# ziyamammadov/conjugate-gradient-pyopencl

Measured on AMD Instinct MI355X. Metric: CG iterations/sec + SpMV effective HBM GB/s (% of 8 TB/s peak), N=10M CSR, higher is better.
Workload: dtype f64; 1 GPU; 3D 7-pt Laplacian 250x200x200 CSR, N=10000000, nnz=69720000, f64, 1 RHS, b=5, x0=0, fixed-iteration CG (fused 4-launch loop); rows=10000000, nnz=69720000, parallelism=1 GPU

## Files before the change

conjugate-gradient-pyopencl_amd/_lib.py:

```python
import ctypes
import os

import numpy as np

_HERE = os.path.dirname(os.path.abspath(__file__))
LIB_PATH = os.path.join(_HERE, "libcgamd.so")
LEGACY_LIB_PATH = os.path.join(_HERE, "liboclcg.so")

F32, F64, C64, C128 = 0, 1, 2, 3
DTYPE_CODE = {np.dtype(np.float32): F32, np.dtype(np.float64): F64,
              np.dtype(np.complex64): C64, np.dtype(np.complex128): C128}
CODE_DTYPE = {v: k for k, v in DTYPE_CODE.items()}

MATRIX_ON_DEVICE, NO_GRAPH, UNFUSED, DIST_GRAPH, DIST_NO_OVERLAP, DIST_P2P, DIST_P2P_STAGED, DIST_SINGLE_REDUCTION, DIST_RESIDENT = 1, 2, 4, 8, 32, 64, 128, 256, 512
HERMITIAN = 16
OK, ERR_INVALID, ERR_NO_DEVICE, ERR_HIP, ERR_ALLOC, ERR_IO, ERR_COMM, ERR_STATE = range(8)


class CgAmdError(RuntimeError):
    def __init__(self, status, message):
        super().__init__(f"cgamd status {status}: {message}")
        self.status = status


# ... 5 lines not shown
    if _lib is not None:
        return _lib
    if os.environ.get("CGAMD_NO_TORCH", "0") != "1":
        try:
            import torch
        except ImportError:
            pass
    if not os.path.exists(LIB_PATH):
        raise ImportError(
            f"{LIB_PATH} not found: the HIP extension is not built. Run `python -c 'import __graft_entry__ as g; "
            f"g.build()'` or `make -C {os.path.join(_HERE, 'csrc')}`. This package has no CPU fallback.")
    lib = ctypes.CDLL(LIB_PATH)
    vp, ci, ll, sz = ctypes.c_void_p, ctypes.c_int, ctypes.c_longlong, ctypes.c_size_t
    pvp = ctypes.POINTER(ctypes.c_void_p)
    sig = {
        "cgamd_last_error": (ctypes.c_char_p, []),
        "cgamd_version": (ci, []),
        "cgamd_dtype_size": (sz, [ci]),
        "cgamd_tune": (ci, [ctypes.c_char_p, ci]),
        "cgamd_device_count": (ci, []),
        "cgamd_device_name": (ci, [ci, ctypes.c_char_p, sz]),
        "cgamd_ctx_create": (ci, [ci, pvp]),
        "cgamd_ctx_destroy": (ci, [vp]),
        "cgamd_ctx_set_stream": (ci, [vp, vp]),
        "cgamd_ctx_stream": (vp, [vp]),
        "cgamd_ctx_device": (ci, [vp]),
        "cgamd_ctx_synchronize": (ci, [vp]),
        "cgamd_malloc": (ci, [vp, sz, pvp]),
        "cgamd_free": (ci, [vp, vp]),
        "cgamd_memcpy_h2d": (ci, [vp, vp, vp, sz]),
        "cgamd_memcpy_d2h": (ci, [vp, vp, vp, sz]),
        "cgamd_memcpy_d2d": (ci, [vp, vp, vp, sz]),
        "cgamd_memset": (ci, [vp, vp, ci, sz]),
        "cgamd_spmv": (ci, [vp, ci, ci, ll, vp, vp, vp, vp, vp, ci]),
        "cgamd_vdot": (ci, [vp, ci, ci, vp, vp, vp, ci]),
        "cgamd_axpy": (ci, [vp, ci, ci, vp, vp, vp, ci, ci]),
        "cgamd_aypx": (ci, [vp, ci, ci, vp, vp, vp, ci]),
        "cgamd_sub": (ci, [vp, ci, ci, vp, vp, vp, ci]),
        "cgamd_solver_create": (ci, [vp, ci, ci, ll, vp, vp, vp, ci, ci, pvp]),
        "cgamd_solver_create_batched": (ci, [vp, ci, ci, ll, vp, vp, vp, ci, ci, pvp]),
        "cgamd_solver_systems": (ci, [vp]),
        "cgamd_solver_hermitian": (ci, [vp]),
        "cgamd_solver_hermitian_scalars": (ci, [vp, vp, vp]),
        "cgamd_solver_destroy": (ci, [vp]),
        "cgamd_solver_set_rhs": (ci, [vp, vp, vp, ci]),
        "cgamd_solver_set_preconditioner": (ci, [vp, vp, ci]),
        "cgamd_solver_set_preconditioner_tridiag": (ci, [vp, vp, vp, vp, ci]),
        "cgamd_solver_set_preconditioner_tridiag_strided": (ci, [vp, ci, vp, vp, vp, ci]),
        "cgamd_solver_set_preconditioner_line": (ci, [vp, ci]),
        "cgamd_solver_set_preconditioner_jacobi": (ci, [vp]),
        "cgamd_solver_set_preconditioner_batched": (ci, [vp, vp, ci]),
        "cgamd_solver_set_preconditioner_batched_jacobi": (ci, [vp]),
        "cgamd_solver_set_preconditioner_batched_line": (ci, [vp, ci]),
        "cgamd_solver_set_preconditioner_multigrid": (ci, [vp, ci, ci, ci, ci, ctypes.c_double, ci]),
        "cgamd_solver_mg_levels": (ci, [vp]),
        "cgamd_solver_mg_level": (ci, [vp, ci, ctypes.POINTER(ll)]),
        "cgamd_solver_mg_level_matrix": (ci, [vp, ci, vp, vp, vp]),
        "cgamd_solver_mg_apply": (ci, [vp, vp, vp]),
        "cgamd_solver_set_preconditioner_amg": (ci, [vp, ci, ctypes.c_double, ci, ctypes.c_double, ci]),
        "cgamd_solver_mg_aggregates": (ci, [vp, ci, vp, ctypes.POINTER(ci)]),
        "cgamd_solver_preconditioner_source": (ci, [vp]),
        "cgamd_solver_iterate": (ci, [vp, ci]),
        "cgamd_solver_iterate_timed": (ci, [vp, ci, ctypes.POINTER(ctypes.c_float), ctypes.POINTER(ctypes.c_float)]),
        "cgamd_solver_get_x": (ci, [vp, vp, ci]),
        "cgamd_solver_history": (ci, [vp, vp, ci]),
        "cgamd_solver_iterations_done": (ci, [vp]),
        "cgamd_solver_vector": (vp, [vp, ci]),
        "cgamd_solver_ld": (ci, [vp]),
        "cgamd_solver_solve": (ci, [vp, vp, vp, ci, vp]),
        "cgamd_solver_spmv": (ci, [vp, vp, vp, ci]),
        "cgamd_solver_spmm_rowmajor": (ci, [vp, vp, vp, ci]),
        "cgamd_last_spmv_form": (ci, [ctypes.POINTER(ci), ci]),
        "cgamd_solver_dot_partials": (ci, [vp, vp, ll, ctypes.POINTER(ci)]),
        "cgamd_solver_step_plan": (ci, [vp, ctypes.POINTER(ci), ci]),
        "cgamd_solver_step_state": (ci, [vp, ci, vp, ll, ctypes.POINTER(ll)]),
        "cgamd_solver_layout": (ci, [vp]),
        "cgamd_solver_loop_launches": (ci, [vp]),
        "cgamd_solver_x_lag": (ci, [vp]),
        "cgamd_solver_index_codes": (ci, [vp]),
        "cgamd_solver_value_codes": (ci, [vp]),
        "cgamd_solver_joint_codes": (ci, [vp]),
        "cgamd_solver_row_codes": (ci, [vp]),
        "cgamd_solver_row_pipe": (ci, [vp]),
        "cgamd_solver_iterate_tol": (ci, [vp, ci, ctypes.c_double, ctypes.POINTER(ci)]),
        "cgamd_solver_iterate_until": (ci, [vp, ci, ctypes.POINTER(ctypes.c_double), ci, ci, ctypes.POINTER(ci)]),
        "cgamd_solver_replace_residual": (ci, [vp, vp]),
        "cgamd_mixed_create": (ci, [vp, ci, ci, ll, vp, vp, vp, ci, ci, pvp]),
        "cgamd_mixed_destroy": (ci, [vp]),
        "cgamd_mixed_outer": (vp, [vp]),
        "cgamd_mixed_inner": (vp, [vp]),
        "cgamd_mixed_solve": (ci, [vp, vp, vp, ci, ctypes.POINTER(ctypes.c_double), ci, ci, ctypes.c_double, ci, ci, ctypes.POINTER(ci),
                                   ctypes.POINTER(ctypes.c_double), ctypes.POINTER(ci), ctypes.POINTER(ci)]),
        "cgamd_mixed_scales": (ci, [vp, ctypes.POINTER(ctypes.c_double)]),
        "cgamd_transpose": (ci, [vp, ci, ci, ci, vp, vp]),
        "cgamd_solver_spmv_bytes": (ll, [vp]),
        "cgamd_solver_iter_bytes": (ll, [vp, ci]),
        "cgamd_solver_spmv_moved_bytes": (ll, [vp]),
        "cgamd_solver_iter_moved_bytes": (ll, [vp]),
        "cgamd_cg": (ci, [ci, ci, ll, vp, vp, vp, vp, vp, ci, ci, vp, ci]),
        "cgamd_cg_last_timing": (ci, [ctypes.POINTER(ctypes.c_double)]),
        "cgamd_cg_release_cache": (ci, []),
        "cgamd_solver_reload_matrix": (ci, [vp, vp, vp, vp]),
        "cgamd_solver_refresh_values": (ci, [vp, vp, ci]),
        "cgamd_solver_last_refresh": (ci, [vp]),
        "cgamd_solver_graph_captures": (ci, [vp]),
        "cgamd_gen_laplace3d": (ci, [vp, ci, ci, ci, ci, ll, ll, vp, vp, vp, ctypes.POINTER(ll)]),
        "cgamd_gen_poisson2d": (ci, [vp, ci, ci, vp, vp, vp, ctypes.POINTER(ll)]),
        "cgamd_gen_helm_fe_var": (ci, [vp, ci, ci, ctypes.c_double, vp, ctypes.c_double, ci, ci, vp, vp, vp, ctypes.POINTER(ll)]),
        "cgamd_gen_local_rect": (ci, [vp, ci, ci, ctypes.c_double, ctypes.c_double, ctypes.c_double, ctypes.c_double, ci, ci, vp, vp, vp,
                                 ctypes.POINTER(ll)]),
        "cgamd_gen_rhs": (ci, [vp, ci, ci, ci, ctypes.c_double, vp]),
        "cgamd_mm_read": (ci, [ctypes.c_char_p, ctypes.POINTER(ci), ctypes.POINTER(ll), ctypes.POINTER(ci),
                               ctypes.POINTER(ctypes.POINTER(ctypes.c_double)),
                               ctypes.POINTER(ctypes.POINTER(ci)), ctypes.POINTER(ctypes.POINTER(ci))]),
        "cgamd_mm_free": (None, [vp]),
        "cgamd_comm_unique_id": (ci, [vp]),
        "cgamd_dist_create": (ci, [vp, vp, ci, ci, ci, ci, ci, ll, vp, vp, vp, ci, vp, vp, vp, vp, ci, pvp]),
        "cgamd_dist_destroy": (ci, [vp]),
        "cgamd_dist_set_rhs": (ci, [vp, vp, vp]),
        "cgamd_dist_iterate": (ci, [vp, ci]),
        "cgamd_dist_iterate_until": (ci, [vp, ci, ctypes.c_double, ci, ctypes.POINTER(ci)]),
        "cgamd_dist_iterations_done": (ci, [vp]),
        "cgamd_dist_get_x": (ci, [vp, vp]),
        "cgamd_dist_history": (ci, [vp, vp, ci]),
        "cgamd_dist_synchronize": (ci, [vp]),
        "cgamd_dist_set_preconditioner": (ci, [vp, vp]),
        "cgamd_dist_set_preconditioner_jacobi": (ci, [vp]),
        "cgamd_dist_set_preconditioner_line": (ci, [vp, ci]),
        "cgamd_dist_refresh_values": (ci, [vp]),
        "cgamd_dist_last_refresh": (ci, [vp]),
        "cgamd_p2p_mailbox_alloc": (ci, [vp, ll, ci, pvp, vp]),
        "cgamd_p2p_mailbox_free": (ci, [vp, vp]),
        "cgamd_dist_attach_p2p": (ci, [vp, vp, vp, vp]),
        "cgamd_dist_p2p_error": (ci, [vp]),
        "cgamd_dist_enable_resident": (ci, [vp, ll, vp, vp]),
        "cgamd_dist_index_codes": (ci, [vp]),
        "cgamd_dist_loop_launches": (ci, [vp]),
        "cgamd_dist_comm_ranks": (ci, [vp]),
        "cg": (vp, [ci, ci, vp, vp, vp, vp, vp, ci, ci, ci]),
    }
    for name, (res, args) in sig.items():
        fn = getattr(lib, name)
        fn.restype = res
        fn.argtypes = args
    _lib = lib
    return lib


def check(status):
    if status != 0:
        raise CgAmdError(status, load().cgamd_last_error().decode(errors="replace"))


def ptr(a):
    if a is None:
        return None
    if isinstance(a, int):
        return ctypes.c_void_p(a)
    if isinstance(a, np.ndarray):
        return a.ctypes.data_as(ctypes.c_void_p)
    if hasattr(a, "data_ptr"):
        return ctypes.c_void_p(a.data_ptr())
    if hasattr(a, "ptr"):
        return ctypes.c_void_p(a.ptr)
    raise TypeError(f"cannot take the address of {type(a)}")
```

conjugate-gradient-pyopencl_amd/cl.py:

```python
import ctypes
import threading

import numpy as np

from . import _lib
from ._lib import CgAmdError, check, ptr

IS_COMPLEX = True
WAVE_SIZE = 64
LOCAL_SIZE = 4 * WAVE_SIZE


class Device:

    def __init__(self, index):
        self.index = int(index)
        buf = ctypes.create_string_buffer(256)
        check(_lib.load().cgamd_device_name(self.index, buf, 256))
        self.name = buf.value.decode()

    def __repr__(self):
        return f"<Device {self.index}: {self.name}>"


# ... 347 lines not shown

    def mg_apply(self, r):
        r = np.ascontiguousarray(np.asarray(r).reshape(-1), dtype=self.dtype)
        if r.size != self.n_rhs * self.size:
            raise ValueError("mg_apply takes n_rhs * size values")
        rd, zd = DeviceBuffer(self.ctx, hostbuf=r), DeviceBuffer(self.ctx, nbytes=r.nbytes, dtype=self.dtype)
        try:
            check(self._lib.cgamd_solver_mg_apply(self.handle, ptr(rd), ptr(zd)))
            return zd.get()
        finally:
            rd.release()
            zd.release()

    def _set_tridiag(self, m):
        coo = m.tocoo()
        dist = np.unique(np.abs(coo.row.astype(np.int64) - coo.col)[coo.data != 0])
        far = dist[dist > 1]
        if far.size > 1 or (far.size == 1 and 1 in dist):
            raise ValueError("only a diagonal or tridiagonal M is supported: stored non-zeros on |i - j| <= 1, or on |i - j| in "
                             "{0, s} for one stride s (the strided tridiagonal form); M has them at distances "
                             f"{dist[:8].tolist()} (the reference's general spsolve branch is out of scope)")
        n = self.size
        lower, diag, upper = np.zeros(n, self.dtype), np.zeros(n, self.dtype), np.zeros(n, self.dtype)
        diag[:] = m.diagonal(0)
        if far.size == 1:
            s = int(far[0])
            lower[s:] = m.diagonal(-s)
            upper[:-s] = m.diagonal(s)
            check(self._lib.cgamd_solver_set_preconditioner_tridiag_strided(self.handle, s, ptr(lower), ptr(diag), ptr(upper), 0))
            return
        if n > 1:
            lower[1:] = m.diagonal(-1)
            upper[:-1] = m.diagonal(1)
        check(self._lib.cgamd_solver_set_preconditioner_tridiag(self.handle, ptr(lower), ptr(diag), ptr(upper), 0))

    def iterate(self, n_iterations):
        check(self._lib.cgamd_solver_iterate(self.handle, int(n_iterations)))

    def replace_residual(self, r):
        if isinstance(r, np.ndarray):
            buf = DeviceBuffer(self.ctx, hostbuf=np.ascontiguousarray(r.reshape(-1), dtype=self.dtype))
            try:
                check(self._lib.cgamd_solver_replace_residual(self.handle, ptr(buf)))
                self.ctx.synchronize()
            finally:
                buf.release()
            return
        check(self._lib.cgamd_solver_replace_residual(self.handle, ptr(r)))

    def iterate_timed(self, n_iterations):
        a, b = ctypes.c_float(), ctypes.c_float()
        check(self._lib.cgamd_solver_iterate_timed(self.handle, int(n_iterations), ctypes.byref(a), ctypes.byref(b)))
        return a.value, b.value

    def x(self, out=None):
        if out is None:
            out = np.empty(self.size * self.n_rhs, dtype=self.dtype)
        on_device = not isinstance(out, np.ndarray)
        check(self._lib.cgamd_solver_get_x(self.handle, ptr(out), int(on_device)))
        if on_device:
            self.ctx.synchronize()
        return out

    def iterations_done(self):
        return int(self._lib.cgamd_solver_iterations_done(self.handle))

    def history(self):
        n = self._lib.cgamd_solver_iterations_done(self.handle) + 1
        out = np.empty((n, self.n_rhs), dtype=self.dtype)
        got = self._lib.cgamd_solver_history(self.handle, ptr(out), n)
        if got < 0:
            check(-got)
        return out[:got]

    def solve(self, b, x0=None, n_iterations=10):
        self.set_rhs(b, x0)
        self.iterate(n_iterations)
        return self.x(), self.history()

    def spmv(self, x, y, fused_dot=False):
        check(self._lib.cgamd_solver_spmv(self.handle, ptr(x), ptr(y), int(fused_dot)))

    SPMV_FAMILIES = ("stream", "rowblock", "vc", "vcp", "chunked", "spmm", "batched")
    SPMV_FAMILIES_EXTRA = ("rowcode",)
    SPMV_FORM_FIELDS = ("family", "vec", "width", "index_bits", "value_codes", "nt", "fused", "wide", "grid", "partials")

    def last_spmv_form(self):
        out = (ctypes.c_int * len(self.SPMV_FORM_FIELDS))()
        got = self._lib.cgamd_last_spmv_form(out, len(out))
        if got < 0:
            check(-got)
        form = dict(zip(self.SPMV_FORM_FIELDS, (int(v) for v in out)))
        names = self.SPMV_FAMILIES + self.SPMV_FAMILIES_EXTRA
        form["family"] = names[form["family"]] if form["family"] >= 0 else None
        return form

    def dot_partials(self):
        per = ctypes.c_int()
        probe = np.empty(1, np.complex128)
        self._lib.cgamd_solver_dot_partials(self.handle, ptr(probe), 0, ctypes.byref(per))
        out = np.empty((self.n_rhs, per.value), dtype=np.complex128 if self.dtype.kind == "c" else np.float64)
        check(self._lib.cgamd_solver_dot_partials(self.handle, ptr(out), out.size, ctypes.byref(per)))
        return out

    STEP_PLAN_FIELDS = ("n", "ld", "vgrid", "n_partials", "kdq", "krr", "fold", "alpha2", "vec", "vec_nt", "x_lag")
    STEP_STATES = ("part_rr", "part_rz", "alpha", "beta", "delta", "rho2", "iter")

    def step_plan(self):
        out = (ctypes.c_int * len(self.STEP_PLAN_FIELDS))()
        got = self._lib.cgamd_solver_step_plan(self.handle, out, len(out))
        if got < 0:
            check(-got)
        return dict(zip(self.STEP_PLAN_FIELDS, (int(v) for v in out)))

    def step_state(self, which):
        idx = self.STEP_STATES.index(which)
        count = ctypes.c_longlong()
        probe = np.empty(1, np.complex128)
        self._lib.cgamd_solver_step_state(self.handle, idx, ptr(probe), 0, ctypes.byref(count))
        if count.value < 1:
            check(self._lib.cgamd_solver_step_state(self.handle, idx, ptr(probe), 0, ctypes.byref(count)))
        acc = np.complex128 if self.dtype.kind == "c" else np.float64
        out = np.empty(count.value, dtype=acc if idx < 2 else np.intc if idx == 6 else self.dtype)
        check(self._lib.cgamd_solver_step_state(self.handle, idx, ptr(out), out.size, ctypes.byref(count)))
        if idx == 6:
            return int(out[0])
        return out.reshape((self.n_rhs, -1) if idx < 2 else (2, self.n_rhs) if idx == 5 else (self.n_rhs,))

    def spmm_rowmajor(self, x, y, n_rhs):
        check(self._lib.cgamd_solver_spmm_rowmajor(self.handle, ptr(x), ptr(y), int(n_rhs)))

    def vector(self, which):
        return self._lib.cgamd_solver_vector(self.handle, {"x": 0, "r": 1, "d": 2, "q": 3}[which])

    @property
    def ld(self):
        return self._lib.cgamd_solver_ld(self.handle)

    @property
    def preconditioner_source(self):
        return self._lib.cgamd_solver_preconditioner_source(self.handle)

    @property
    def spmv_bytes(self):
        return self._lib.cgamd_solver_spmv_bytes(self.handle)

    @property
    def index_codes(self):
        return self._lib.cgamd_solver_index_codes(self.handle)

    @property
    def value_codes(self):
        return self._lib.cgamd_solver_value_codes(self.handle)

    @property
    def joint_codes(self):
        return self._lib.cgamd_solver_joint_codes(self.handle)

    @property
    def row_codes(self):
        return self._lib.cgamd_solver_row_codes(self.handle)

    @property
    def row_pipe(self):
        return self._lib.cgamd_solver_row_pipe(self.handle)

    def iter_bytes(self, fused=False):
        return self._lib.cgamd_solver_iter_bytes(self.handle, int(fused))

    @property
    def spmv_moved_bytes(self):
        return self._lib.cgamd_solver_spmv_moved_bytes(self.handle)

    @property
    def iter_moved_bytes(self):
        return self._lib.cgamd_solver_iter_moved_bytes(self.handle)

    def close(self):
        if getattr(self, "handle", None) and getattr(self.ctx, "handle", None) and not getattr(self, "_borrowed", False):
            self._lib.cgamd_solver_destroy(self.handle)
        self.handle = None

    def __del__(self):
        try:
            self.close()
        except Exception:
            pass


    def solve_tol(self, b, x0=None, tol=1e-5, maxit=1000, check_every=8):
        if self.n_rhs != 1:
            raise ValueError("solve_tol handles one right-hand side")
        if self._lib.cgamd_solver_loop_launches(self.handle) < 2:
            self.set_rhs(b, x0)
            run_ = ctypes.c_int(0)
            st = self._lib.cgamd_solver_iterate_tol(self.handle, int(maxit), float(tol), ctypes.byref(run_))
            if st == 0:
                return self.x(), int(run_.value), self.history()
            if st != _lib.ERR_STATE:
                check(st)

        its = self._run_to_tol(b, x0, tol, int(maxit), int(check_every))
        return self.x(), its, self.history()

    def _run_to_tol(self, b, x0, tol, maxit, check_every):
        self.set_rhs(b, x0)
        done, step, its = 0, max(1, check_every), maxit
        while done < maxit:
            s_ = min(step, maxit - done)
            self.iterate(s_)
            done += s_
            norms = np.sqrt(np.abs(self.history()[:, 0]))
            hit = np.nonzero(~(norms[1:] >= tol))[0]
            if hit.size:
                its = int(hit[0]) + 1
                break
            cur, start = float(norms[-1]), float(norms[-1 - s_])
            step = max(1, check_every)
            if 0.0 < cur < start and tol > 0:
                togo = np.log(tol / cur) / (np.log(cur / start) / s_)
                if togo < 2 * step:
                    step = max(1, int(togo / 2))
        if self.iterations_done() != its:
            self.set_rhs(b, x0)
            self.iterate(its)
        return its

    def _tolerances(self, tol):
        t = np.ascontiguousarray(np.asarray(tol, dtype=np.float64).reshape(-1))
        if t.size not in (1, self.n_rhs):
            raise ValueError(f"tol must be a scalar or have n_rhs = {self.n_rhs} entries, got {t.size}")
        if not np.all(t > 0):
            raise ValueError("every tolerance must be positive")
        return t

    def iterate_until(self, tol, maxit, check_every=8):
        t = self._tolerances(tol)
        if int(maxit) < 0 or int(check_every) < 0:
            raise ValueError("maxit and check_every must not be negative")
        its = np.zeros(self.n_rhs, dtype=np.intc)
        check(self._lib.cgamd_solver_iterate_until(self.handle, int(maxit), t.ctypes.data_as(ctypes.POINTER(ctypes.c_double)), int(t.size),
                                                   int(check_every), its.ctypes.data_as(ctypes.POINTER(ctypes.c_int))))
        return its

    def solve_until(self, b, x0=None, tol=1e-5, maxit=1000, check_every=8):
        self._tolerances(tol)
        self.set_rhs(b, x0)
        its = self.iterate_until(tol, maxit, check_every)
# ... 263 lines not shown
```

conjugate-gradient-pyopencl_amd/csrc/api.cpp:

```cpp
#include <atomic>
#include <pthread.h>

#include <chrono>
#include <cstdio>
#include <cstdlib>
#include <cstring>
#include <mutex>
#include <string>
#include <vector>

#include "../../include/clcg.h"
#include "cgamd_internal.h"

namespace cgamd {
static thread_local std::string g_err;
void set_error(const std::string &msg) { g_err = msg; }
int fail(int status, const std::string &msg) {
    g_err = msg;
    return status;
}
}
using namespace cgamd;

extern "C" {

const char *cgamd_last_error(void) { return g_err.c_str(); }
int cgamd_version(void) { return 100; }
size_t cgamd_dtype_size(int dtype) { return dtype_size(dtype); }

static std::atomic<unsigned long long> g_tune_generation{1};

int cgamd_tune(const char *key, int value) {
    if (!key) return fail(CGAMD_ERR_INVALID, "tune: null key");
    const std::string k(key);
    bool known = true;
    if (k == "dev.x_lag" && value != -1 && value != 0 && value != 1 && value != 2 && value != 4 && value != 8)
        return fail(CGAMD_ERR_INVALID, "tune: dev.x_lag takes -1 (default rule), 0 or 1 (off), 2, 4 or 8");
    if (k == "dev.row_pipe" && value != 0 && value != 1 && value != 2 && value != 4)
        return fail(CGAMD_ERR_INVALID, "tune: dev.row_pipe takes 0 (default rule), 1, 2 or 4");
    g_tune_generation.fetch_add(1, std::memory_order_relaxed);
    tune_set([&](Tuning &g_tune) {
    if (k == "index_codes") g_tune.index_codes = value;
    else if (k == "index_codes16") g_tune.index_codes16 = value;
    else if (k == "index_codes_min_mb") g_tune.index_codes_min_mb = value;
    else if (k == "resident") g_tune.resident = value;
    else if (k == "resident_min") g_tune.resident_min = value;
    else if (k == "resident_wide") g_tune.resident_wide = value;
    else if (k == "resident_wide_min") g_tune.resident_wide_min = value;
    else if (k == "resident_claim_ms") g_tune.resident_claim_ms = value;
    else if (k == "two_launch") g_tune.two_launch = value;
    else if (k == "spmm_rowmajor") g_tune.spmm_rowmajor = value;
    else if (k == "pad_rows") g_tune.pad_rows = value;
    else if (k == "spmv_nt") g_tune.spmv_nt = value;
    else if (k == "vec_nt") g_tune.vec_nt = value;
    else if (k == "spmv_cycle") g_tune.spmv_cycle = value;
    else if (k == "vec_grid") g_tune.vec_grid = value;
    else if (k == "dev.no_fold_alpha") g_tune.dev_no_fold_alpha = value;
    else if (k == "dev.x_lag") g_tune.dev_x_lag = value;
    else if (k == "dev.x_lag_dnt") g_tune.dev_x_lag_dnt = value;
    else if (k == "dev.generic_spmv") g_tune.dev_generic_spmv = value;
    else if (k == "dev.value_codes") g_tune.value_codes = value;
    else if (k == "dev.vc_pipe") g_tune.dev_vc_pipe = value;
    else if (k == "dev.joint_codes") g_tune.dev_joint_codes = value;
    else if (k == "dev.row_codes") g_tune.dev_row_codes = value;
    else if (k == "dev.row_codes_min_mb") g_tune.dev_row_codes_min_mb = value;
    else if (k == "dev.row_pipe") g_tune.dev_row_pipe = value;
    else if (k == "dev.resident_lock") g_tune.resident_lock = value;
    else if (k == "dev.slab_cus") g_tune.slab_cus = value;
    else if (k == "dev.slab_trim") g_tune.slab_trim = value;
    else if (k == "dev.resident_test_short_grid") g_tune.resident_test_short_grid = value;
    else if (k == "dev.resident_wide_rpt") g_tune.resident_wide_rpt = value;
    else if (k == "dev.resident_window") g_tune.resident_window = value;
    else if (k == "dev.vec_ppt") g_tune.vec_ppt = value;
    else if (k == "dev.spmv_unroll") g_tune.spmv_unroll = value;
    else if (k == "dev.spmv_grid") g_tune.spmv_grid = value;
    else if (k == "dev.spmv_slice_kb") g_tune.spmv_slice_kb = value;
    else if (k == "dev.spmv_chunk_kb") g_tune.spmv_chunk_kb = value;
    else if (k == "dev.spmv_chunked") g_tune.spmv_chunked = value;
    else if (k == "dev.spmm_ynt") g_tune.spmm_ynt = value;
    else if (k == "dev.spmm_group") g_tune.spmm_group = value;
    else if (k == "dev.spmm_rb") g_tune.spmm_rb = value;
    else if (k == "dev.spmm_wgs") g_tune.spmm_wgs = value;
    else if (k == "dev.spmm_lead") g_tune.spmm_lead = value;
    else if (k == "dev.spmm_wide_max") g_tune.spmm_wide_max = value;
    else if (k == "dev.line_host_route") g_tune.dev_line_host_route = value;
    else known = false;
    });
    if (!known) return fail(CGAMD_ERR_INVALID, "tune: unknown key " + k);
    return CGAMD_OK;
}

int cgamd_device_count(void) {
    int n = 0;
    hipError_t e = hipGetDeviceCount(&n);
    if (e != hipSuccess) {
        fail(CGAMD_ERR_NO_DEVICE, std::string("hipGetDeviceCount: ") + hipGetErrorString(e));
        return -CGAMD_ERR_NO_DEVICE;
    }
    return n;
}

int cgamd_device_name(int device, char *buf, size_t buflen) {
    if (!buf || !buflen) return fail(CGAMD_ERR_INVALID, "device_name: null buffer");
    hipDeviceProp_t p;
    CG_HIP(hipGetDeviceProperties(&p, device));
    snprintf(buf, buflen, "%s (%s, %d CUs)", p.name, p.gcnArchName, p.multiProcessorCount);
    return CGAMD_OK;
}

int cgamd_ctx_create(int device, cgamd_ctx **out) {
    if (!out) return fail(CGAMD_ERR_INVALID, "ctx_create: out is NULL");
    *out = nullptr;
    int n = cgamd_device_count();
    if (n <= 0) return fail(CGAMD_ERR_NO_DEVICE, "no HIP device available (this library has no CPU fallback)");
    thread_hip_setup();
    if (device < 0 || device >= n) return fail(CGAMD_ERR_INVALID, "ctx_create: device index out of range");
    CG_HIP(hipSetDevice(device));
    cgamd_ctx *c = new cgamd_ctx();
    c->device = device;
    hipError_t e = hipStreamCreateWithFlags(&c->stream, hipStreamNonBlocking);
    if (e != hipSuccess) {
        delete c;
        return fail(CGAMD_ERR_HIP, std::string("hipStreamCreate: ") + hipGetErrorString(e));
    }
    c->own_stream = true;
    *out = c;
    return CGAMD_OK;
}

int cgamd_ctx_destroy(cgamd_ctx *c) {
    if (!c) return CGAMD_OK;
    (void)hipSetDevice(c->device);
    if (c->partials) (void)hipFree(c->partials);
    if (c->own_stream && c->stream) (void)hipStreamDestroy(c->stream);
    delete c;
    return CGAMD_OK;
}

int cgamd_ctx_set_stream(cgamd_ctx *c, void *stream) {
    if (!c) return fail(CGAMD_ERR_INVALID, "ctx is NULL");
    if (c->own_stream && c->stream) {
        (void)hipStreamSynchronize(c->stream);
        (void)hipStreamDestroy(c->stream);
    }
    c->own_stream = false;
    c->stream = static_cast<hipStream_t>(stream);
    return CGAMD_OK;
}
void *cgamd_ctx_stream(cgamd_ctx *c) { return c ? (void *)c->stream : nullptr; }
// ... 307 lines not shown
```

conjugate-gradient-pyopencl_amd/csrc/cgamd_internal.h:

```cpp
#pragma once
#include <hip/hip_runtime.h>
#include <cstddef>
#include <cstdint>
#include <string>
#include <vector>

#include "../../include/cgamd.h"

namespace cgamd {

void set_error(const std::string &msg);
int fail(int status, const std::string &msg);
#define CG_HIP(expr)                                                                         \
    do {                                                                                     \
        hipError_t e__ = (expr);                                                             \
        if (e__ != hipSuccess)                                                               \
            return ::cgamd::fail(e__ == hipErrorNoDevice || e__ == hipErrorInvalidDevice     \
                                     ? CGAMD_ERR_NO_DEVICE : CGAMD_ERR_HIP,                  \
                                 std::string(#expr) + ": " + hipGetErrorString(e__));        \
    } while (0)

inline size_t dtype_size(int dt) { return dt == 0 ? 4 : dt == 1 ? 8 : dt == 2 ? 8 : dt == 3 ? 16 : 0; }
inline size_t acc_size(int dt) { return (dt == 0 || dt == 1) ? 8 : 16; }
inline bool aligned16(const void *p) { return (reinterpret_cast<uintptr_t>(p) & 15u) == 0; }

constexpr int kBlock = 256;
constexpr int kMaxGrid = 2048;
constexpr int kQuadsPerThread = 2;

struct SpmvPlan {
    int grid = 0;
    int row_blocks = 0;
    int max_span = 0;
    int kind = 0;
    int chunk_span[5] = {0, 0, 0, 0, 0};
    bool wide = false;
    int max_row = 0;
    int max_quad = 0;
    int lpr = 1;
    int n_partials = 0;
    int fold_max = 0;
    int nt = 1;
    int vec_nt = 3;
    const unsigned char *codes = nullptr;
    const int *dict = nullptr;
    const int *codes_for = nullptr;
    bool codes16 = false;
    const unsigned char *vcodes = nullptr;
    const void *vdict = nullptr;
    const void *vcodes_for = nullptr;
    const unsigned char *jcodes = nullptr;
    const int *jdict_off = nullptr;
    const void *jdict_val = nullptr;
    const unsigned char *rcodes = nullptr;
    const int *rdict_len = nullptr;
    const int *rdict_off = nullptr;
    const void *rdict_val = nullptr;
    int n_patterns = 0;
    const int *rcodes_for = nullptr;
};
SpmvPlan make_spmv_plan(int n);
int compute_spmv_plan(const int *ptr_dev, const int *cols_dev, int n, int *scratch_dev, hipStream_t st, SpmvPlan *plan);
int validate_csr_device(int n, long long nnz, int ncols, const int *ptr_dev, const int *cols_dev, const int *index_dev, int n_index,
                        int index_bound, int *scratch_dev, hipStream_t st);
int build_index_codes(int n, long long nnz, const int *ptr_dev, const int *cols_dev, hipStream_t st, unsigned char **codes_out,
                      int **dict_out, int *distinct_out);
int build_joint_codes(int dtype, long long nnz, const unsigned char *codes, const unsigned char *vcodes, const int *dict, const void *vdict,
                      hipStream_t st, unsigned char **jcodes_out, int **joff_out, void **jval_out, int *n_pairs);
constexpr size_t row_dict_off_at(size_t value_size) { return 256 * 8 * value_size; }
constexpr size_t row_dict_len_at(size_t value_size) { return row_dict_off_at(value_size) + 256 * 8 * sizeof(int); }
constexpr size_t row_dict_bytes(size_t value_size) { return row_dict_len_at(value_size) + 256 * sizeof(int); }
constexpr size_t row_dict_jmap_at(size_t value_size) { return row_dict_bytes(value_size); }
constexpr size_t row_dict_alloc_bytes(size_t value_size) { return row_dict_jmap_at(value_size) + 256 * 8; }
int build_row_codes(int dtype, int n, int n_user, const int *ptr_dev, const unsigned char *jcodes, const int *joff, const void *jval, hipStream_t st,
                    unsigned char **rcodes_out, void **rdict_out, int *n_patterns, int *n_user_patterns);
int build_value_codes(int dtype, long long nnz, const void *vals_dev, hipStream_t st, unsigned char **vcodes_out, void **vdict_out, int *n_values);
int refresh_value_dicts(int dtype, long long nnz, const void *vals_dev, const unsigned char *vcodes, void *vdict, int n_pairs, const int *joff,
                        void *jval, int n_patterns, void *rdict, hipStream_t st, bool *kept);
int build_index_codes16(int n, long long nnz, const int *ptr_dev, const int *cols_dev, hipStream_t st, unsigned char **codes_out, int **base_out);
void finalize_spmv_plan(SpmvPlan *plan, int dtype, int nrhs, int n, long long nnz, const void *vals, const int *cols);
constexpr int kChunkBytes = 32 * 1024;
constexpr int kMaxChunkBytes = 48 * 1024;
constexpr int kMaxSpmmSliceBytes = 64 * 1024;
constexpr int kMaxSliceBytes = 40 * 1024;

struct Tuning {
    int index_codes = 1;
    int index_codes16 = 1;
    int index_codes_min_mb = 32;
    int resident = 1;
    int resident_min = 8;
    int resident_wide = 1;
    int resident_wide_min = 16;
    int resident_claim_ms = 200;
    int two_launch = 1;
    int spmm_rowmajor = 1;
    int pad_rows = 1;
    int spmv_nt = -1;
    int vec_nt = -1;
    int spmv_cycle = 64;
    int vec_grid = 0;
    int dev_no_fold_alpha = 0;
    int dev_x_lag = -1;
    int dev_x_lag_dnt = 1;
    int value_codes = 1;
    int dev_joint_codes = 1;
    int dev_row_codes = 1;
    int dev_row_codes_min_mb = 32;
    int dev_row_pipe = 0;
    int dev_vc_pipe = 1;
    int dev_generic_spmv = 0;
    int resident_lock = 1;
    int slab_trim = -1;
    int slab_cus = 0;
    int resident_test_short_grid = 0;
    int resident_wide_rpt = 0;
    int resident_window = 1;
    int vec_ppt = 0;
    int spmv_unroll = 0;
    int spmv_grid = 0;
    int spmv_slice_kb = 0;
    int spmv_chunk_kb = 0;
    int spmv_chunked = 1;
    int spmm_ynt = -1;
    int spmm_group = 0;
    int spmm_rb = 0;
    int spmm_wgs = 0;
    int spmm_lead = 0;
    int spmm_wide_max = -1;
    int dev_line_host_route = 0;
};
inline int row_pipe_depth(int knob, size_t value_bytes) { return knob == 1 || knob == 2 || knob == 4 ? knob : value_bytes <= 4 ? 4 : 1; }
extern Tuning g_tune;
Tuning tune_snapshot();
const Tuning &tune();
}
#include <functional>
namespace cgamd {
void tune_set(const std::function<void(Tuning &)> &edit);
void set_kernel_event_pair(hipEvent_t *pair);
void thread_hip_setup();
struct TuneScope {
    const Tuning *prev;
    explicit TuneScope(const Tuning *t);
    ~TuneScope();
};
int vec_grid(long long n_elems_per_rhs, int dtype, int nrhs = 1);

constexpr int kSpmvFormFields = 10;
void last_spmv_form(int *out, int n_out);
void record_spmv_form(const int *fields);
int launch_spmv(int dtype, const SpmvPlan &plan, int n, long long nnz, const void *vals, const int *ptr,
                const int *cols, const void *x, long long ldx, void *y, long long ldy, int nrhs,
                const void *dvec, void *partials, hipStream_t st, const int *rb_list = nullptr, int rb_count = 0);
int launch_spmv_batched(int dtype, const SpmvPlan &plan, int n, long long nnz, int nsys, const void *vals, const int *ptr, const int *cols,
                        const void *x, long long ldx, void *y, long long ldy, const void *dvec, void *partials, hipStream_t st);
int launch_halo_flags(int n, const int *ptr, const int *cols, int n_local, int row_blocks, int *flag, hipStream_t st);
int launch_dot_partials(int dtype, int n, const void *a, const void *b, long long ld, int nrhs, void *partials,
                        int grid, hipStream_t st);
int launch_reduce_to_value(int dtype, const void *partials, int grid, int nrhs, void *result, hipStream_t st);
int launch_axpy(int dtype, int n, const void *x, void *y, long long ld, const void *a, int sign, int nrhs, hipStream_t st);
struct CgStop;
int launch_aypx(int dtype, int n, const void *x, void *y, long long ld, const void *a, int nrhs, hipStream_t st, const CgStop *stop = nullptr);
int launch_sub(int dtype, int n, const void *a, const void *b, void *res, long long ld, int nrhs, hipStream_t st);
int launch_axpy2_dot(int dtype, int n, const void *d, void *x, const void *q, void *r, long long ld,
                     const void *alpha, int nrhs, void *partials, int grid, hipStream_t st, int vec_nt = 3, const CgStop *stop = nullptr);

struct CgScalars {
    void *alpha = nullptr;
    void *beta = nullptr;
    void *delta = nullptr;
    void *history = nullptr;
    int *iter = nullptr;
    int history_cap = 0;
    void *stage = nullptr;
    unsigned *ticket = nullptr;
    int kdq = 0, krr = 0;
    const void *pcg_m = nullptr;
    void *pcg_rho2 = nullptr;
};
struct CgStop {
    int *nactive = nullptr;
    const double *tol = nullptr;
    int *stop = nullptr;
    int *live = nullptr;
};
#pragma GCC visibility push(hidden)
struct StopRun {
    void *rec = nullptr;
    CgStop view;
    int nr = 0;
    int *pin = nullptr;
    int *stopped = nullptr;
    hipEvent_t ev[2] = {nullptr, nullptr};
    bool armed = false;
    int enqueued = 0;
    bool active = true;
};
int stop_run_alloc(StopRun &sr, int nr);
int stop_run_arm(StopRun &sr, const double *tol, int nTol, hipStream_t st);
int stop_run_chunks(StopRun &sr, int maxIterations, int chunk, hipStream_t st, const std::function<int(int)> &enqueue);
int stop_run_read(StopRun &sr, hipStream_t st);
void stop_run_free(StopRun &sr);
#pragma GCC visibility pop
int launch_axpy_dot(int dtype, int n, const void *q, void *r, long long ld, const void *alpha, int nrhs, void *partials, int grid,
                    hipStream_t st, int vec_nt = 3, const CgStop *stop = nullptr);
int launch_axpy_dot_alpha(int dtype, int n, const void *q, void *r, long long ld, const void *part_dq, int P, const CgScalars &sc,
                          int nrhs, void *partials, int grid, hipStream_t st, const CgStop *stop = nullptr);
int launch_aypx_beta_x(int dtype, int n, const void *x, void *y, void *xs, long long ld, const void *partials, int P, int nrhs,
                       const CgScalars &sc, hipStream_t st, int vec_nt = 3, const CgStop *stop = nullptr);
constexpr int kLagMax = 8;
constexpr int lag_alpha_slot(int j, int lag) { return (j + 1) % lag; }
int launch_aypx_beta_out(int dtype, int n, const void *r, const void *d_in, void *d_out, long long ld, const void *partials, int P,
                         int nrhs, const CgScalars &sc, hipStream_t st, int vec_nt = 3);
int launch_aypx_beta_xlag(int dtype, int n, int lag, const void *r, void *const *dirs, void *xs, long long ld, const void *partials, int P,
// ... 310 lines not shown
```

conjugate-gradient-pyopencl_amd/csrc/index_codes.hip:

```cpp
#include "cgamd_internal.h"
#include "device_types.h"
#include "device_mem.h"
#include "spmv_device.h"
#include "reduce_device.h"
#include "launch_util.h"

#include <hip/hip_ext.h>

#include <algorithm>
#include <functional>
#include <mutex>
#include <vector>

namespace cgamd {

constexpr int kDictSlots = 1024;
constexpr int kDictEmpty = -2147483647 - 1;
CG_DEV unsigned dict_hash(int d) { return ((unsigned)d * 2654435761u) >> 22; }
__global__ __launch_bounds__(256) void index_offsets_kernel(int n, const int *__restrict__ ptr, const int *__restrict__ cols,
                                                            int *table, int *count) {
    for (long long row = blockIdx.x * 256LL + threadIdx.x; row < n; row += 256LL * gridDim.x) {
        if (__hip_atomic_load(count, __ATOMIC_RELAXED, __HIP_MEMORY_SCOPE_AGENT) > 256) return;
        int last = kDictEmpty;
        for (int j = ptr[row], e = ptr[row + 1]; j < e; ++j) {
            const int d = cols[j] - (int)row;
            if (d == last) continue;
            last = d;
            unsigned h = dict_hash(d);
            int probes = 0;
            for (; probes < kDictSlots; ++probes, h = (h + 1) & (kDictSlots - 1)) {
                int v = __hip_atomic_load(table + h, __ATOMIC_RELAXED, __HIP_MEMORY_SCOPE_AGENT);
                if (v == kDictEmpty) {
                    v = atomicCAS(table + h, kDictEmpty, d);
                    if (v == kDictEmpty) { atomicAdd(count, 1); break; }
                }
                if (v == d) break;
            }
            if (probes == kDictSlots) { atomicAdd(count, kDictSlots); return; }
        }
    }
}
__global__ __launch_bounds__(256) void index_encode_kernel(int n, const int *__restrict__ ptr, const int *__restrict__ cols,
                                                           const int *__restrict__ table, const unsigned char *__restrict__ slot_code,
                                                           unsigned char *__restrict__ codes) {
    __shared__ int stab[kDictSlots];
    __shared__ unsigned char scode[kDictSlots];
    for (int i = threadIdx.x; i < kDictSlots; i += 256) { stab[i] = table[i]; scode[i] = slot_code[i]; }
    __syncthreads();
    for (long long row = blockIdx.x * 256LL + threadIdx.x; row < n; row += 256LL * gridDim.x) {
        for (int j = ptr[row], e = ptr[row + 1]; j < e; ++j) {
            const int d = cols[j] - (int)row;
            unsigned h = dict_hash(d);
            while (stab[h] != d) h = (h + 1) & (kDictSlots - 1);
            codes[j] = scode[h];
        }
    }
}

int build_index_codes(int n, long long nnz, const int *ptr_dev, const int *cols_dev, hipStream_t st, unsigned char **codes_out,
                      int **dict_out, int *distinct_out) {
    *codes_out = nullptr;
    *dict_out = nullptr;
    *distinct_out = 0;
    if (n <= 0 || nnz <= 0) return CGAMD_OK;
    int *work = nullptr;
    CG_HIP(hipMalloc((void **)&work, (kDictSlots + 64 + 256) * sizeof(int) + kDictSlots));
    std::vector<int> table(kDictSlots + 1, kDictEmpty);
    table[kDictSlots] = 0;
    hipError_t e = hipMemcpyAsync(work, table.data(), (kDictSlots + 1) * sizeof(int), hipMemcpyHostToDevice, st);
    int g = (int)std::min<long long>((n + 255LL) / 256, 8192);
    if (e == hipSuccess) {
        hipLaunchKernelGGL(index_offsets_kernel, dim3(g), dim3(256), 0, st, n, ptr_dev, cols_dev, work, work + kDictSlots);
        e = hipMemcpyAsync(table.data(), work, (kDictSlots + 1) * sizeof(int), hipMemcpyDeviceToHost, st);
    }
    if (e == hipSuccess) e = hipStreamSynchronize(st);
    if (e != hipSuccess) { (void)hipFree(work); return fail(CGAMD_ERR_HIP, std::string("build_index_codes: ") + hipGetErrorString(e)); }
    const int distinct = table[kDictSlots];
    if (distinct < 1 || distinct > 256) { (void)hipFree(work); return CGAMD_OK; }
    std::vector<int> dict;
    for (int i = 0; i < kDictSlots; ++i)
        if (table[i] != kDictEmpty) dict.push_back(table[i]);
    std::sort(dict.begin(), dict.end());
    std::vector<unsigned char> slot_code(kDictSlots, 0);
    for (int i = 0; i < kDictSlots; ++i)
        if (table[i] != kDictEmpty) slot_code[i] = (unsigned char)(std::lower_bound(dict.begin(), dict.end(), table[i]) - dict.begin());
    dict.resize(256, dict[0]);
    unsigned char *codes = nullptr;
    int *dict_dev = nullptr;
// ... 443 lines not shown
    for (long long p = (long long)blockIdx.x * 256 + threadIdx.x; p < packs; p += stride) {
        if (__hip_atomic_load(flag, __ATOMIC_RELAXED, __HIP_MEMORY_SCOPE_AGENT)) return;
        const uint4 w = *reinterpret_cast<const uint4 *>(vals + p * E);
        if constexpr (sizeof(T) == 4) {
            unsigned c;
            __builtin_memcpy(&c, vcodes + p * 4, 4);
            refresh_claim(w.x, c & 255, stab, table, flag);
            refresh_claim(w.y, (c >> 8) & 255, stab, table, flag);
            refresh_claim(w.z, (c >> 16) & 255, stab, table, flag);
            refresh_claim(w.w, c >> 24, stab, table, flag);
        } else {
            unsigned short c;
            __builtin_memcpy(&c, vcodes + p * 2, 2);
            refresh_claim(((unsigned long long)w.y << 32) | w.x, c & 255u, stab, table, flag);
            refresh_claim(((unsigned long long)w.w << 32) | w.z, c >> 8, stab, table, flag);
        }
    }
    const long long j = packs * E + threadIdx.x;
    if (blockIdx.x == 0 && j < nnz) refresh_claim(value_key(vals[j]), vcodes[j], stab, table, flag);
}
template <typename T>
__global__ __launch_bounds__(256) void refresh_dicts_kernel(const unsigned long long *__restrict__ table, T *vdict, int n_pairs, const int *__restrict__ jmap,
                                                            T *jval, int n_patterns, const int *__restrict__ rlen,
                                                            const unsigned char *__restrict__ rjmap, T *rval) {
    __shared__ T sv[256], sj[256];
    const int t = threadIdx.x;
    const unsigned long long key = table[t];
    T v = vdict[t];
    if (key != kVEmpty) {
        if constexpr (sizeof(T) == 4) { const unsigned b = (unsigned)key; __builtin_memcpy(&v, &b, 4); }
        else __builtin_memcpy(&v, &key, 8);
        vdict[t] = v;
    }
    sv[t] = v;
    __syncthreads();
    if (!jval) return;
    if (t < n_pairs) { sj[t] = sv[jmap[t] & 255]; jval[t] = sj[t]; }
    __syncthreads();
    if (!rval) return;
    for (int p = t; p < n_patterns * 8; p += 256)
        if ((p & 7) < rlen[p >> 3]) rval[p] = sj[rjmap[p]];
}
template <typename T>
static int refresh_value_dicts_impl(long long nnz, const void *vals, const unsigned char *vcodes, void *vdict, int n_pairs, const int *joff, void *jval,
                                    int n_patterns, void *rdict, hipStream_t st, bool *kept) {
    char *scratch = nullptr;
    const size_t tb = sizeof(unsigned long long) * 256;
    CG_HIP(hipMalloc((void **)&scratch, tb + 16));
    auto *table = reinterpret_cast<unsigned long long *>(scratch);
    int *flag = reinterpret_cast<int *>(scratch + tb);
    int h = 1;
    hipError_t e = hipMemsetAsync(table, 0xff, tb, st);
    if (e == hipSuccess) e = hipMemsetAsync(flag, 0, 16, st);
    const long long packs = nnz / (long long)(16 / sizeof(T));
    const int grid = (int)std::max<long long>(1, std::min<long long>((packs + 255) / 256, kMaxGrid));
    if (e == hipSuccess) {
        hipLaunchKernelGGL((refresh_check_kernel<T>), dim3(grid), dim3(256), 0, st, nnz, static_cast<const T *>(vals), vcodes, table, flag);
        e = hipMemcpyAsync(&h, flag, sizeof(int), hipMemcpyDeviceToHost, st);
    }
    if (e == hipSuccess) e = hipStreamSynchronize(st);
    if (e == hipSuccess && h == 0) {
        char *rd = static_cast<char *>(rdict);
        hipLaunchKernelGGL((refresh_dicts_kernel<T>), dim3(1), dim3(256), 0, st, table, static_cast<T *>(vdict), n_pairs, joff ? joff + 256 : nullptr,
                           static_cast<T *>(jval), n_patterns, rd ? reinterpret_cast<const int *>(rd + row_dict_len_at(sizeof(T))) : nullptr,
                           rd ? reinterpret_cast<const unsigned char *>(rd + row_dict_jmap_at(sizeof(T))) : nullptr, reinterpret_cast<T *>(rd));
        e = hipGetLastError();
        if (e == hipSuccess) e = hipStreamSynchronize(st);
    }
    (void)hipFree(scratch);
    if (e != hipSuccess) return fail(CGAMD_ERR_HIP, std::string("refresh_value_dicts: ") + hipGetErrorString(e));
    *kept = h == 0;
    return CGAMD_OK;
}
int refresh_value_dicts(int dtype, long long nnz, const void *vals_dev, const unsigned char *vcodes, void *vdict, int n_pairs, const int *joff,
                        void *jval, int n_patterns, void *rdict, hipStream_t st, bool *kept) {
    *kept = false;
    if (nnz <= 0 || !vcodes || !vdict || dtype == CGAMD_C128 || !aligned16(vals_dev)) return CGAMD_OK;
    if (!joff || !jval) { joff = nullptr; jval = nullptr; rdict = nullptr; }
    if (dtype == CGAMD_F32) return refresh_value_dicts_impl<float>(nnz, vals_dev, vcodes, vdict, n_pairs, joff, jval, n_patterns, rdict, st, kept);
    if (dtype == CGAMD_F64) return refresh_value_dicts_impl<double>(nnz, vals_dev, vcodes, vdict, n_pairs, joff, jval, n_patterns, rdict, st, kept);
    return refresh_value_dicts_impl<float2>(nnz, vals_dev, vcodes, vdict, n_pairs, joff, jval, n_patterns, rdict, st, kept);
}

}
```

conjugate-gradient-pyopencl_amd/csrc/solver.cpp:

```cpp
#include <algorithm>
#include <cmath>
#include <complex>
#include <cstring>
#include <vector>

#include "cgamd_internal.h"
#include "launch_util.h"

using namespace cgamd;

struct cgamd_solver {
    Tuning tune;
    cgamd_ctx *ctx = nullptr;
    int dtype = 0, n = 0, nrhs = 1, flags = 0;
    int n_user = 0;
    int nsys = 0;
    bool herm = false;
    bool own_ptr = false;
    long long nnz = 0;
    void *vals = nullptr;
    int *ptr = nullptr, *cols = nullptr;
    bool own_matrix = false;
    std::vector<int> ptr_host;
    SpmvPlan plan;
    int vgrid = 1;
    void *x = nullptr, *r = nullptr, *d = nullptr, *q = nullptr, *b = nullptr;
    void *slab = nullptr;
    void *part_dq = nullptr, *part_rr = nullptr;
    size_t part_dq_cap = 0;
    void *mdiag = nullptr, *part_rz = nullptr, *rho2 = nullptr;
    bool tri_on = false;
    TriLaunch tri;
    void *tri_coef = nullptr, *tri_part = nullptr;
    int *tri_cstart = nullptr;
    int pre_source = 0, pre_kind = 0, pre_stride = 0;
    MgHierarchy *mg = nullptr;
    MgParams mg_params;
    CgScalars sc;
    bool rhs_set = false;
    int iters = 0;
    hipGraphExec_t g1[2] = {nullptr, nullptr}, gU[2] = {nullptr, nullptr};
    hipGraph_t g1g[2] = {nullptr, nullptr}, gUg[2] = {nullptr, nullptr};
    int U = 8;
    bool graph_failed = false;
    bool rm_ok = false, rm = false;
    int rm_nwg = 0, rm_vgrid = 0;
    size_t part_rr_cap = 0;
    int *rm_pace = nullptr;
    hipEvent_t *ev_pair = nullptr;
    bool fused2 = false;
    void *d2 = nullptr;
    int x_lag = 1;
    void *dlag = nullptr;
    size_t dlag_pitch = 0;
    int dlag_bufs = 0;
    bool res_ok = false;
    ResidentPlan res;
    void *res_sync = nullptr;
    int n_cus = 0;
    ResidentWidePlan resw;
    void *resw_sync = nullptr;
    unsigned char *codes = nullptr;
    int *dict = nullptr;
    int n_offsets = 0;
    unsigned char *vcodes = nullptr;
    void *vdict = nullptr;
    int n_values = 0;
    unsigned char *jcodes = nullptr;
    int *jdict_off = nullptr;
    void *jdict_val = nullptr;
    int n_pairs = 0;
    unsigned char *rcodes = nullptr;
    void *rdict = nullptr;
    int n_patterns = 0, n_user_patterns = 0;
    double tol_req = 0.;
    bool tol_served = false, tol_stopped = false;
    StopRun stop;
    bool until_mode = false, until_stopped = false;
    hipGraphExec_t gT = nullptr;
    hipGraph_t gTg = nullptr;
    int gT_len = 0;
    int last_refresh = 0;
    int captures = 0;
};

static void destroy_graphs(cgamd_solver *s) {
    for (int p = 0; p < 2; ++p) {
        if (s->g1[p]) (void)hipGraphExecDestroy(s->g1[p]);
        if (s->gU[p]) (void)hipGraphExecDestroy(s->gU[p]);
        if (s->g1g[p]) (void)hipGraphDestroy(s->g1g[p]);
        if (s->gUg[p]) (void)hipGraphDestroy(s->gUg[p]);
        s->g1[p] = s->gU[p] = nullptr;
        s->g1g[p] = s->gUg[p] = nullptr;
    }
    if (s->gT) (void)hipGraphExecDestroy(s->gT);
    if (s->gTg) (void)hipGraphDestroy(s->gTg);
    s->gT = nullptr; s->gTg = nullptr; s->gT_len = 0;
}

static void drop_multigrid(cgamd_solver *s) {
    if (s->mg) mg_free(s->mg);
    s->mg = nullptr;
}

static int dmalloc(void **p, size_t bytes, const char *what) {
    hipError_t e = hipMalloc(p, bytes ? bytes : 16);
    if (e != hipSuccess)
        return fail(CGAMD_ERR_ALLOC, std::string("hipMalloc(") + what + ", " + std::to_string(bytes) + " B): " + hipGetErrorString(e));
    return CGAMD_OK;
}

static int validate_csr_host(int n, long long nnz, const int *ptr, const int *cols) {
    if (ptr[0] != 0) return fail(CGAMD_ERR_INVALID, "CSR: aPointers[0] != 0");
    for (int i = 0; i < n; ++i)
        if (ptr[i + 1] < ptr[i]) return fail(CGAMD_ERR_INVALID, "CSR: aPointers not monotone at row " + std::to_string(i));
    if (ptr[n] != nnz) return fail(CGAMD_ERR_INVALID, "CSR: aPointers[size] != nonZeros");
    for (long long j = 0; j < nnz; ++j)
        if (cols[j] < 0 || cols[j] >= n) return fail(CGAMD_ERR_INVALID, "CSR: column index out of range at entry " + std::to_string(j));
    return CGAMD_OK;
}

static void *dbuf(cgamd_solver *s, int k) { return (s->fused2 && !s->until_mode && (k & 1)) ? s->d2 : s->d; }
static bool precond_set(const cgamd_solver *s) { return s->mdiag != nullptr || s->tri_on || s->mg != nullptr; }
static long long m_pitch(const cgamd_solver *s) { return s->nsys ? s->n : 0; }
static bool fused2_now(const cgamd_solver *s) { return s->fused2 && !s->rm && !precond_set(s) && !(s->flags & CGAMD_UNFUSED) && !s->until_mode; }

static int handle_spmv(cgamd_solver *s, int n, const void *x, long long ldx, void *y, long long ldy, const void *dvec, void *partials,
                       hipStream_t st) {
    if (s->nsys)
        return launch_spmv_batched(s->dtype, s->plan, n, s->nnz, s->nsys, s->vals, s->ptr, s->cols, x, ldx, y, ldy, dvec, partials, st);
    return launch_spmv(s->dtype, s->plan, n, s->nnz, s->vals, s->ptr, s->cols, x, ldx, y, ldy, s->nrhs, dvec, partials, st);
}

static int enqueue_spmv(cgamd_solver *s, int k, hipStream_t st, void *dvec = nullptr) {
    const int dt = s->dtype, n = s->n, nr = s->nrhs;
    const bool fused2 = fused2_now(s);
    const bool ext = s->ev_pair && !fused2 && !s->rm && nr == 1 && s->plan.kind == 5 && !s->nsys;
    if (s->ev_pair && !ext) CG_HIP(hipEventRecord(s->ev_pair[0], st));
    if (ext) set_kernel_event_pair(s->ev_pair);
    int rc;
    if (fused2)
        rc = launch_spmv_fused(dt, s->plan, n, s->nnz, s->vals, s->ptr, s->cols, dbuf(s, k), dbuf(s, k + 1), s->r, s->q, nr, s->part_dq,
                               s->part_rr, s->vgrid, s->sc, st);
    else if (s->rm) rc = launch_spmm_rm(dt, n, s->nnz, s->vals, s->ptr, s->cols, s->d, s->q, nr, s->part_dq, s->plan.max_quad, s->rm_pace, st);
    else if ((s->flags & CGAMD_UNFUSED) && !s->tri_on && !(s->nsys && s->mdiag)) rc = handle_spmv(s, n, s->d, n, s->q, n, nullptr, nullptr, st);
    else if (s->herm) rc = handle_spmv(s, n, s->d, n, s->q, n, s->d2, s->part_dq, st);
    else rc = handle_spmv(s, n, dvec ? dvec : s->d, n, s->q, n, dvec ? dvec : s->d, s->part_dq, st);
    set_kernel_event_pair(nullptr);
    if (rc) return rc;
    if (s->ev_pair && !ext) CG_HIP(hipEventRecord(s->ev_pair[1], st));
    return CGAMD_OK;
}

struct TriPartials { void *rz, *rr; };
static TriPartials tri_partials(const cgamd_solver *s) {
    return {s->tri_part, static_cast<char *>(s->tri_part) + acc_size(s->dtype) * (size_t)s->tri.grid * s->nrhs};
// ... 64 lines not shown
        return launch_pcg_aypx_beta_z(dt, n, s->d, s->q, n, s->part_rz, s->part_rr, s->vgrid, nr, s->sc, s->rho2, s->x, st, g);
    }
    if (s->tri_on) {
        if ((rc = enqueue_spmv(s, k, st))) return rc;
        if ((rc = launch_cg_alpha(dt, s->part_dq, s->plan.n_partials, nr, s->sc, st, g))) return rc;
        if ((rc = enqueue_tri_sweep(s, true, s->q, s->q, st, g))) return rc;
        const TriPartials p = tri_partials(s);
        return launch_pcg_aypx_beta_z(dt, n, s->d, s->q, n, p.rz, p.rr, s->tri.grid, nr, s->sc, s->rho2, s->x, st, g);
    }
    if (s->mdiag) {
        if ((rc = enqueue_spmv(s, k, st))) return rc;
        if ((rc = launch_cg_alpha(dt, s->part_dq, s->plan.n_partials, nr, s->sc, st, g))) return rc;
        if ((rc = launch_pcg_axpy2_dot2(dt, false, n, s->d, s->x, s->q, s->r, s->mdiag, n, s->sc.alpha, nr, s->part_rz, s->part_rr,
                                        s->vgrid, st, m_pitch(s), g))) return rc;
        return launch_pcg_aypx_beta(dt, n, s->r, s->d, s->mdiag, n, s->part_rz, s->part_rr, s->vgrid, nr, s->sc, s->rho2, s->x, st, m_pitch(s), g);
    }
    if (!(s->flags & CGAMD_UNFUSED)) {
        if ((rc = enqueue_spmv(s, k, st))) return rc;
        const bool fold = fold_alpha_ok(s->plan.n_partials, s->plan.fold_max);
        if (!fold && (rc = launch_cg_alpha(dt, s->part_dq, s->plan.n_partials, nr, s->sc, st, g))) return rc;
        if (fold) rc = launch_axpy_dot_alpha(dt, n, s->q, s->r, n, s->part_dq, s->plan.n_partials, s->sc, nr, s->part_rr, s->vgrid, st, g);
        else rc = launch_axpy_dot(dt, n, s->q, s->r, n, s->sc.alpha, nr, s->part_rr, s->vgrid, st, s->plan.vec_nt, g);
        if (rc) return rc;
        return launch_aypx_beta_x(dt, n, s->r, s->d, s->x, n, s->part_rr, s->vgrid, nr, s->sc, st, s->plan.vec_nt, g);
    }
    if ((rc = enqueue_spmv(s, k, st))) return rc;
    if ((rc = launch_dot_partials(dt, n, s->d, s->q, n, nr, s->part_rr, s->vgrid, st))) return rc;
    if ((rc = launch_cg_alpha(dt, s->part_rr, s->vgrid, nr, s->sc, st))) return rc;
    if ((rc = launch_axpy(dt, n, s->d, s->x, n, s->sc.alpha, 1, nr, st))) return rc;
    if ((rc = launch_axpy(dt, n, s->q, s->r, n, s->sc.alpha, 0, nr, st))) return rc;
    if ((rc = launch_dot_partials(dt, n, s->r, s->r, n, nr, s->part_rr, s->vgrid, st))) return rc;
    if ((rc = launch_cg_beta(dt, s->part_rr, s->vgrid, nr, s->sc, st))) return rc;
    return launch_aypx(dt, n, s->r, s->d, n, s->sc.beta, nr, st);
}

static void apply_wide_order(cgamd_solver *s) {
    if (s->nsys) return;
    const int E = (int)(16 / dtype_size(s->dtype));
    const bool wide = s->resw.ok && !s->tri_on && !s->mg && (!s->res_ok || precond_set(s));
    const int kdq = wide ? kResWideBlocksPerRpt * s->resw.rpt : 0, krr = wide ? kdq / E : 0;
    const int vgrid = wide ? (s->n / E + kBlock - 1) / kBlock : vec_grid(s->n, s->dtype, s->nrhs);
    const int fold_max = 0;
    if (kdq == s->sc.kdq && krr == s->sc.krr && vgrid == s->vgrid && fold_max == s->plan.fold_max) return;
    destroy_graphs(s);
    s->sc.kdq = kdq; s->sc.krr = krr; s->vgrid = vgrid; s->plan.fold_max = fold_max;
    s->fused2 = !s->herm && fused2_ok(s->plan, s->dtype, s->nrhs, s->vals, s->cols);
}

static int setup_resident_wide_plan(cgamd_solver *s) {
    s->resw.ok = false;
    if (tune().resident_wide == 0 || tune().resident == 0 || (s->flags & CGAMD_UNFUSED)) return CGAMD_OK;
    if (s->rm_ok && tune().spmm_rowmajor >= 2) return CGAMD_OK;
    if (!aligned16(s->x) || !aligned16(s->r) || !aligned16(s->d) || !aligned16(s->d2)) return CGAMD_OK;
    if (s->plan.kind != 5 && s->plan.kind != 6) return CGAMD_OK;
    if (s->n % (int)(16 / dtype_size(s->dtype)) != 0) return CGAMD_OK;
    if (!s->n_cus) CG_HIP(hipDeviceGetAttribute(&s->n_cus, hipDeviceAttributeMultiprocessorCount, s->ctx->device));
    ResidentWidePlan wp;
    if (int rc = resident_wide_plan(s->dtype, s->n, s->nnz, s->nrhs, s->n_cus, s->ptr, s->cols, s->sc.iter, s->ctx->stream, &wp, s->fused2)) return rc;
    if (!wp.ok) return CGAMD_OK;
    if ((size_t)((s->n / (int)(16 / dtype_size(s->dtype)) + kBlock - 1) / kBlock) > s->part_rr_cap) return CGAMD_OK;
    if (s->resw_sync && wp.sync_bytes > s->resw.sync_bytes) { (void)hipFree(s->resw_sync); s->resw_sync = nullptr; }
    if (!s->resw_sync)
        if (int rc = dmalloc(&s->resw_sync, wp.sync_bytes, "wide resident sync words")) return rc;
    s->resw = wp;
    s->rm_ok = false;
    return CGAMD_OK;
}

static void drop_value_codes(cgamd_solver *s) {
    if (s->vcodes) { (void)hipFree(s->vcodes); s->vcodes = nullptr; }
    if (s->vdict) { (void)hipFree(s->vdict); s->vdict = nullptr; }
    s->plan.vcodes = nullptr; s->plan.vdict = nullptr; s->plan.vcodes_for = nullptr;
    s->n_values = 0;
    if (s->jcodes) { (void)hipFree(s->jcodes); s->jcodes = nullptr; }
    if (s->jdict_off) { (void)hipFree(s->jdict_off); s->jdict_off = nullptr; }
    if (s->jdict_val) { (void)hipFree(s->jdict_val); s->jdict_val = nullptr; }
    s->plan.jcodes = nullptr; s->plan.jdict_off = nullptr; s->plan.jdict_val = nullptr;
    s->n_pairs = 0;
    if (s->rcodes) { (void)hipFree(s->rcodes); s->rcodes = nullptr; }
    if (s->rdict) { (void)hipFree(s->rdict); s->rdict = nullptr; }
    s->plan.rcodes = nullptr; s->plan.rdict_len = nullptr; s->plan.rdict_off = nullptr; s->plan.rdict_val = nullptr; s->plan.n_patterns = 0;
    s->plan.rcodes_for = nullptr;
    s->n_patterns = 0; s->n_user_patterns = 0;
}
static bool value_codes_apply(const cgamd_solver *s) {
    return s->codes && !s->plan.codes16 && !s->nsys && s->tune.value_codes && s->plan.kind == 5 && s->dtype != CGAMD_C128;
}
static int setup_value_codes(cgamd_solver *s) {
    if (!value_codes_apply(s)) return CGAMD_OK;
    const size_t matrix_bytes = (size_t)s->nnz * (dtype_size(s->dtype) + 4);
    if (int rc = build_value_codes(s->dtype, s->nnz, s->vals, s->ctx->stream, &s->vcodes, &s->vdict, &s->n_values)) return rc;
    if (s->vcodes) { s->plan.vcodes = s->vcodes; s->plan.vdict = s->vdict; s->plan.vcodes_for = s->vals; }
    if (!s->vcodes || !s->tune.dev_joint_codes) return CGAMD_OK;
    if (int rc = build_joint_codes(s->dtype, s->nnz, s->codes, s->vcodes, s->dict, s->vdict, s->ctx->stream, &s->jcodes, &s->jdict_off,
                                   &s->jdict_val, &s->n_pairs)) return rc;
    if (s->jcodes) { s->plan.jcodes = s->jcodes; s->plan.jdict_off = s->jdict_off; s->plan.jdict_val = s->jdict_val; }
    const size_t vsz = dtype_size(s->dtype);
    if (s->jcodes && s->nrhs == 1 && s->plan.kind == 5 && s->plan.max_row > 0 && s->plan.max_row <= 7 && s->tune.dev_row_codes &&
        s->tune.dev_row_codes_min_mb >= 0 && matrix_bytes > ((size_t)s->tune.dev_row_codes_min_mb << 20) &&
        (unsigned long long)s->n * vsz < (1ULL << 30)) {
        if (int rc = build_row_codes(s->dtype, s->n, s->n_user, s->ptr, s->jcodes, s->jdict_off, s->jdict_val, s->ctx->stream, &s->rcodes,
                                     &s->rdict, &s->n_patterns, &s->n_user_patterns)) return rc;
        if (s->rcodes) {
            const char *rd = static_cast<const char *>(s->rdict);
            s->plan.rcodes = s->rcodes; s->plan.rdict_val = rd; s->plan.n_patterns = s->n_patterns;
            s->plan.rdict_off = reinterpret_cast<const int *>(rd + row_dict_off_at(vsz));
            s->plan.rdict_len = reinterpret_cast<const int *>(rd + row_dict_len_at(vsz));
            s->plan.rcodes_for = s->ptr;
        }
    }
    return CGAMD_OK;
}

static int setup_index_codes(cgamd_solver *s) {
    if (s->codes) { (void)hipFree(s->codes); s->codes = nullptr; }
    if (s->dict) { (void)hipFree(s->dict); s->dict = nullptr; }
    s->plan.codes = nullptr; s->plan.dict = nullptr; s->plan.codes_for = nullptr; s->plan.codes16 = false;
    s->n_offsets = 0;
    drop_value_codes(s);
    const size_t matrix_bytes = (size_t)s->nnz * (dtype_size(s->dtype) + 4);
    if (s->resw.ok && !(s->flags & CGAMD_NO_GRAPH) && s->tune.index_codes < 2) return CGAMD_OK;
    if (!s->tune.index_codes || s->nrhs != 1 || (s->plan.kind != 5 && s->plan.kind != 7) || s->tune.index_codes_min_mb < 0 ||
        matrix_bytes <= ((size_t)s->tune.index_codes_min_mb << 20))
        return CGAMD_OK;
    if (int rc = build_index_codes(s->n, s->nnz, s->ptr, s->cols, s->ctx->stream, &s->codes, &s->dict, &s->n_offsets)) return rc;
    if (s->codes) {
        s->plan.codes = s->codes; s->plan.dict = s->dict; s->plan.codes_for = s->cols; s->plan.codes16 = false;
        return setup_value_codes(s);
    }
    if (s->tune.index_codes16 == 0) return CGAMD_OK;
    if (int rc = build_index_codes16(s->n, s->nnz, s->ptr, s->cols, s->ctx->stream, &s->codes, &s->dict)) return rc;
    if (s->codes) { s->plan.codes = s->codes; s->plan.dict = s->dict; s->plan.codes_for = s->cols; s->plan.codes16 = true; s->n_offsets = 65536; }
    return CGAMD_OK;
}

static int setup_resident_local(cgamd_solver *s);
static int setup_resident(cgamd_solver *s) {
    const int rc = setup_resident_local(s);
    apply_wide_order(s);
    return rc;
}
static int setup_resident_one_xcd(cgamd_solver *s);
static int setup_resident_local(cgamd_solver *s) {
    s->res_ok = false;
    s->resw.ok = false;
    if (s->herm) return CGAMD_OK;
    if (int rc = setup_resident_one_xcd(s)) return rc;
    if (s->res_ok && !s->mdiag) return CGAMD_OK;
    return setup_resident_wide_plan(s);
}
static int setup_resident_one_xcd(cgamd_solver *s) {
    if (!s->fused2 || tune().resident == 0 || s->n > 65536) return CGAMD_OK;
    std::vector<int> tmp;
    const int *ph = s->ptr_host.size() == (size_t)s->n + 1 ? s->ptr_host.data() : nullptr;
    if (!ph) {
        tmp.resize((size_t)s->n + 1);
        CG_HIP(hipMemcpyAsync(tmp.data(), s->ptr, tmp.size() * 4, hipMemcpyDeviceToHost, s->ctx->stream));
        CG_HIP(hipStreamSynchronize(s->ctx->stream));
        ph = tmp.data();
    }
    if (!s->n_cus) CG_HIP(hipDeviceGetAttribute(&s->n_cus, hipDeviceAttributeMultiprocessorCount, s->ctx->device));
    ResidentPlan rp;
    if (!aligned16(s->x) || !aligned16(s->r) || !aligned16(s->d) || !aligned16(s->d2)) return CGAMD_OK;
    int max_window = 0;
    if (s->n % (int)(16 / dtype_size(s->dtype)) == 0)
        if (int rc = resident_max_window(s->dtype, s->n, s->ptr, s->cols, s->sc.iter, s->ctx->stream, &max_window)) return rc;
    if (!resident_plan(s->dtype, s->n, vec_grid(s->n, s->dtype, s->nrhs), s->plan.n_partials, s->n_cus, ph, max_window, &rp)) return CGAMD_OK;
    if (s->res_sync && rp.sync_bytes > s->res.sync_bytes) { (void)hipFree(s->res_sync); s->res_sync = nullptr; }
    if (!s->res_sync)
        if (int rc = dmalloc(&s->res_sync, rp.sync_bytes, "resident sync words")) return rc;
    s->res = rp;
    s->res_ok = true;
    return CGAMD_OK;
}

constexpr int kXLagDefault = 4;
static void setup_x_lag(cgamd_solver *s) {
    const int knob = s->tune.dev_x_lag;
    int lag = knob >= 0 ? std::max(knob, 1) : (fold_alpha_ok(s->plan.n_partials, s->plan.fold_max) || s->resw.ok ? 1 : kXLagDefault);
    if (s->nsys || s->herm || (s->flags & (CGAMD_UNFUSED | CGAMD_NO_GRAPH)) || lag > kLagMax || s->U % lag != 0) lag = 1;
    if (lag - 2 > s->dlag_bufs) {
        if (s->dlag) { (void)hipStreamSynchronize(s->ctx->stream); (void)hipFree(s->dlag); s->dlag = nullptr; s->dlag_bufs = 0; }
        s->dlag_pitch = ((size_t)s->n * s->nrhs * dtype_size(s->dtype) + 4095) & ~(size_t)4095;
        if (hipMalloc(&s->dlag, s->dlag_pitch * (size_t)(lag - 2)) == hipSuccess) s->dlag_bufs = lag - 2;
        else { (void)hipGetLastError(); s->dlag = nullptr; lag = 1; }
    }
    if (lag != s->x_lag) destroy_graphs(s);
    s->x_lag = lag;
}

static int capture(cgamd_solver *s, int k0, int iters, hipGraph_t *g, hipGraphExec_t *ge, bool guarded = false) {
// ... 189 lines not shown
    return fail(CGAMD_ERR_STATE, std::string(who) + ": the handle runs the conjugated recurrence (CGAMD_HERMITIAN), " + why);
}
constexpr const char *kHermNoLines = "whose preconditioner is diagonal: the line sweeps form the unconjugated r.z and r.r";
static int line_from_matrix(cgamd_solver *s, const std::string &who, int stride);
static int jacobi_from_matrix(cgamd_solver *s, const std::string &who);
static int batched_line_from_matrix(cgamd_solver *s, const std::string &who, int stride);
static int batched_jacobi_from_matrix(cgamd_solver *s, const std::string &who);
static int multigrid_from_matrix(cgamd_solver *s, const std::string &who, const MgParams &p);
static int step_not_capturing(cgamd_solver *s, const char *who);
static int rebuild_from_matrix(cgamd_solver *s, const std::string &who) {
    if (s->pre_kind == 3) return multigrid_from_matrix(s, who, s->mg_params);
    return s->pre_kind == 1 ? jacobi_from_matrix(s, who) : line_from_matrix(s, who, s->pre_stride);
}

int cgamd_solver_reload_matrix(cgamd_solver *s, const void *aValues, const int *aPointers, const int *aCols) {
    if (!s || !aPointers || (s->nnz > 0 && (!aValues || !aCols))) return fail(CGAMD_ERR_INVALID, "reload_matrix: null argument");
    if (!s->own_matrix) return fail(CGAMD_ERR_STATE, "reload_matrix: the handle borrows a device matrix");
    TuneScope ts(&s->tune);
    CG_HIP(hipSetDevice(s->ctx->device));
    if (int rc = validate_csr_host(s->n_user, s->nnz, aPointers, aCols)) return rc;
    hipStream_t st = s->ctx->stream;
    const size_t vs = dtype_size(s->dtype);
    s->rhs_set = false;
    if (s->nnz) {
        CG_HIP(hipMemcpyAsync(s->vals, aValues, (size_t)s->nnz * (s->nsys ? (size_t)s->nsys : 1) * vs, hipMemcpyHostToDevice, st));
        CG_HIP(hipMemcpyAsync(s->cols, aCols, (size_t)s->nnz * 4, hipMemcpyHostToDevice, st));
    }
    const bool same_ptr = s->ptr_host.size() == (size_t)s->n + 1 && memcmp(s->ptr_host.data(), aPointers, ((size_t)s->n_user + 1) * 4) == 0;
    if (!same_ptr) {
        CG_HIP(hipMemcpyAsync(s->ptr, aPointers, ((size_t)s->n_user + 1) * 4, hipMemcpyHostToDevice, st));
        std::copy(aPointers, aPointers + s->n_user + 1, s->ptr_host.begin());
        destroy_graphs(s);
        s->plan = make_spmv_plan(s->n);
        if (int rc = compute_spmv_plan(s->ptr, s->cols, s->n, s->sc.iter, st, &s->plan)) return rc;
        finalize_spmv_plan(&s->plan, s->dtype, s->nrhs, s->n, s->nnz, s->vals, s->cols);
        if ((size_t)std::max(s->plan.grid, s->plan.row_blocks) > s->part_dq_cap) return fail(CGAMD_ERR_STATE, "reload_matrix: partial buffer too small");
        if (s->rm_ok) s->rm_nwg = spmm_rm_grid(s->dtype, s->nrhs, s->n, s->plan.max_quad, true);
        s->fused2 = !s->herm && fused2_ok(s->plan, s->dtype, s->nrhs, s->vals, s->cols);
        if (s->nsys) finalize_batched_plan(s);
    }
    if (s->nsys) {
        CG_HIP(hipStreamSynchronize(st));
        if (s->pre_source >= 2) {
            const int rc = s->pre_kind == 1 ? batched_jacobi_from_matrix(s, "reload_matrix") : batched_line_from_matrix(s, "reload_matrix", s->pre_stride);
            if (rc) {
                const std::string why = cgamd_last_error();
                (void)diag_impl(s, nullptr, 0);
                return fail(rc, why);
            }
        }
        return CGAMD_OK;
    }
    if (int rc = setup_resident(s)) return rc;
    {
        const bool had = s->codes != nullptr;
        if (had) destroy_graphs(s);
        if (int rc = setup_index_codes(s)) return rc;
        if (!had && s->codes) destroy_graphs(s);
    }
    setup_x_lag(s);
    CG_HIP(hipStreamSynchronize(st));
    if (s->pre_source >= 2) {
        const int rc = rebuild_from_matrix(s, "reload_matrix");
        if (rc) {
            const std::string why = cgamd_last_error();
            (void)diag_impl(s, nullptr, 0);
            return fail(rc, why);
        }
    }
    return CGAMD_OK;
}

static int refresh_codes(cgamd_solver *s) {
    s->last_refresh = 0;
    if (!value_codes_apply(s) || s->nnz <= 0) return CGAMD_OK;
    if (s->vcodes) {
        bool kept = false;
        if (int rc = refresh_value_dicts(s->dtype, s->nnz, s->vals, s->vcodes, s->vdict, s->n_pairs, s->jcodes ? s->jdict_off : nullptr,
                                         s->jcodes ? s->jdict_val : nullptr, s->n_patterns, s->rcodes ? s->rdict : nullptr, s->ctx->stream, &kept)) {
            destroy_graphs(s);
            drop_value_codes(s);
            return rc;
        }
        if (kept) { s->last_refresh = 1; return CGAMD_OK; }
    }
    const bool had = s->vcodes != nullptr;
    if (had) destroy_graphs(s);
    drop_value_codes(s);
    const int rc = setup_value_codes(s);
    if (!had && s->vcodes) destroy_graphs(s);
    if (rc) { drop_value_codes(s); return rc; }
    s->last_refresh = s->vcodes ? 2 : 3;
    return CGAMD_OK;
}
int cgamd_solver_refresh_values(cgamd_solver *s, const void *aValues, int on_device) {
    if (!s) return fail(CGAMD_ERR_INVALID, "refresh_values: solver is NULL");
    if (s->own_matrix && !aValues) return fail(CGAMD_ERR_INVALID, "refresh_values: the handle owns its matrix: aValues is NULL");
    if (!s->own_matrix && aValues && (aValues != s->vals || !on_device))
        return fail(CGAMD_ERR_INVALID, "refresh_values: the handle borrows its value array (CGAMD_MATRIX_ON_DEVICE): copy the new values into "
                                       "that array and pass NULL (or the array itself, on_device = 1); borrowing another array needs a new handle");
    TuneScope ts(&s->tune);
    CG_HIP(hipSetDevice(s->ctx->device));
    hipStream_t st = s->ctx->stream;
    {
        hipStreamCaptureStatus cs = hipStreamCaptureStatusNone;
        const hipError_t e = hipStreamIsCapturing(st, &cs);
        if (e != hipSuccess) { (void)hipGetLastError(); return fail(CGAMD_ERR_HIP, std::string("refresh_values: hipStreamIsCapturing: ") + hipGetErrorString(e)); }
        if (cs != hipStreamCaptureStatusNone) return fail(CGAMD_ERR_INVALID, "refresh_values: the handle's stream is being captured");
    }
    s->rhs_set = false;
    s->last_refresh = 0;
    CG_HIP(hipStreamSynchronize(st));
    if (s->own_matrix && s->nnz) {
        const size_t bytes = (size_t)s->nnz * (s->nsys ? (size_t)s->nsys : 1) * dtype_size(s->dtype);
        CG_HIP(hipMemcpyAsync(s->vals, aValues, bytes, on_device ? hipMemcpyDeviceToDevice : hipMemcpyHostToDevice, st));
        CG_HIP(hipStreamSynchronize(st));
    }
    if (int rc = refresh_codes(s)) {
        s->last_refresh = -rc;
        if (s->pre_source >= 2) {
            const std::string why = cgamd_last_error();
            (void)diag_impl(s, nullptr, 0);
            return fail(rc, why);
        }
        return rc;
    }
    if (s->pre_source >= 2) {
        int rc;
        if (s->nsys) rc = s->pre_kind == 1 ? batched_jacobi_from_matrix(s, "refresh_values") : batched_line_from_matrix(s, "refresh_values", s->pre_stride);
        else rc = rebuild_from_matrix(s, "refresh_values");
        if (rc) {
            const std::string why = cgamd_last_error();
            (void)diag_impl(s, nullptr, 0);
            return fail(rc, why);
        }
    }
    return CGAMD_OK;
}
int cgamd_solver_last_refresh(cgamd_solver *s) { return s ? s->last_refresh : -CGAMD_ERR_INVALID; }
int cgamd_solver_graph_captures(cgamd_solver *s) { return s ? s->captures : -CGAMD_ERR_INVALID; }

int cgamd_solver_destroy(cgamd_solver *s) {
    if (!s) return CGAMD_OK;
    thread_hip_setup();
    (void)hipSetDevice(s->ctx->device);
    (void)hipStreamSynchronize(s->ctx->stream);
    destroy_graphs(s);
    drop_multigrid(s);
    if (s->own_ptr && s->ptr) (void)hipFree(s->ptr);
    if (s->own_matrix) {
        if (s->vals) (void)hipFree(s->vals);
        if (s->ptr) (void)hipFree(s->ptr);
        if (s->cols) (void)hipFree(s->cols);
    }
    void *bufs[] = {s->slab, s->part_dq, s->part_rr, s->sc.alpha, s->sc.beta, s->sc.delta,
                    s->sc.history, s->sc.iter, s->mdiag, s->part_rz, s->rho2, s->tri_coef, s->tri_part, s->tri_cstart, s->tri.maps, s->sc.stage, s->sc.ticket, s->res_sync, s->resw_sync, s->dlag, s->codes, s->dict, s->rm_pace, s->vcodes, s->vdict, s->jcodes, s->jdict_off, s->jdict_val, s->rcodes, s->rdict};
    for (void *p : bufs)
        if (p) (void)hipFree(p);
    stop_run_free(s->stop);
    delete s;
    return CGAMD_OK;
}

static int set_rhs_impl(cgamd_solver *s, const void *b, const void *x0, int on_device, long long ldb) {
    TuneScope ts(&s->tune);
    CG_HIP(hipSetDevice(s->ctx->device));
    hipStream_t st = s->ctx->stream;
    const size_t vbytes = (size_t)s->n * s->nrhs * dtype_size(s->dtype);
    const hipMemcpyKind kind = on_device ? hipMemcpyDeviceToDevice : hipMemcpyHostToDevice;
    const bool rm = s->rm_ok && !precond_set(s);
    if (rm && (!b || ldb != s->n_user)) return fail(CGAMD_ERR_STATE, "the handle keeps its right-hand sides interleaved (row-major layout)");
    if (rm != s->rm) destroy_graphs(s);
    if (s->until_mode && s->fused2) destroy_graphs(s);
    s->until_mode = s->until_stopped = s->stop.armed = false;
    s->rm = rm;
    int rc;
    if (rm) {
        CG_HIP(hipMemcpyAsync(s->q, b, vbytes, kind, st));
        if ((rc = launch_transpose(s->dtype, s->nrhs, s->n, s->q, s->b, st))) return rc;
        if (x0) {
            CG_HIP(hipMemcpyAsync(s->q, x0, vbytes, kind, st));
            if ((rc = launch_transpose(s->dtype, s->nrhs, s->n, s->q, s->x, st))) return rc;
        } else {
            CG_HIP(hipMemsetAsync(s->x, 0, vbytes, st));
        }
        if ((rc = launch_spmm_rm(s->dtype, s->n, s->nnz, s->vals, s->ptr, s->cols, s->x, s->q, s->nrhs, nullptr, s->plan.max_quad, s->rm_pace, st))) return rc;
        if ((rc = launch_sub(s->dtype, s->n * s->nrhs, s->b, s->q, s->r, (long long)s->n * s->nrhs, 1, st))) return rc;
        CG_HIP(hipMemcpyAsync(s->d, s->r, vbytes, hipMemcpyDeviceToDevice, st));
        if ((rc = launch_rm_dot(s->dtype, s->n, s->nrhs, s->r, s->r, s->part_rr, s->rm_vgrid, st))) return rc;
        if ((rc = launch_cg_delta0(s->dtype, s->part_rr, s->rm_vgrid, s->nrhs, s->sc, st))) return rc;
        if (!on_device) CG_HIP(hipStreamSynchronize(st));
        s->rhs_set = true;
        s->iters = 0;
        return CGAMD_OK;
    }
    if (!b) {
    } else if (s->n != ldb) {
        const size_t vs = dtype_size(s->dtype);
        CG_HIP(hipMemcpy2DAsync(s->b, (size_t)s->n * vs, b, (size_t)ldb * vs, (size_t)s->n_user * vs, (size_t)s->nrhs, kind, st));
        CG_HIP(hipMemsetAsync(s->x, 0, vbytes, st));
        if (x0) CG_HIP(hipMemcpy2DAsync(s->x, (size_t)s->n * vs, x0, (size_t)ldb * vs, (size_t)s->n_user * vs, (size_t)s->nrhs, kind, st));
    } else {
        CG_HIP(hipMemcpyAsync(s->b, b, vbytes, kind, st));
        if (x0) CG_HIP(hipMemcpyAsync(s->x, x0, vbytes, kind, st));
        else CG_HIP(hipMemsetAsync(s->x, 0, vbytes, st));
    }
    if ((rc = handle_spmv(s, s->n, s->x, s->n, s->q, s->n, nullptr, nullptr, st))) return rc;
    if ((rc = launch_sub(s->dtype, s->n, s->b, s->q, s->r, s->n, s->nrhs, st))) return rc;
    if (s->herm) {
        if ((rc = launch_herm_init(s->dtype, s->n, s->r, s->d, s->d2, s->mdiag, m_pitch(s), s->n, s->nrhs, s->part_rz, s->part_rr, s->vgrid, st))) return rc;
        if ((rc = launch_herm_delta0(s->dtype, s->mdiag != nullptr, s->part_rz, s->part_rr, s->vgrid, s->nrhs, s->sc, s->rho2, st))) return rc;
    } else if (s->mg) {
        if ((rc = mg_vcycle(s->mg, s->r, s->d, st))) return rc;
        if ((rc = launch_dot_partials(s->dtype, s->n, s->r, s->r, s->n, s->nrhs, s->part_rr, s->vgrid, st))) return rc;
        if ((rc = launch_dot_partials(s->dtype, s->n, s->r, s->d, s->n, s->nrhs, s->part_rz, s->vgrid, st))) return rc;
        if ((rc = launch_pcg_delta0(s->dtype, s->part_rz, s->part_rr, s->vgrid, s->nrhs, s->sc, s->rho2, st))) return rc;
    } else if (s->tri_on) {
        if ((rc = enqueue_tri_sweep(s, false, nullptr, s->d, st))) return rc;
        const TriPartials p = tri_partials(s);
        if ((rc = launch_pcg_delta0(s->dtype, p.rz, p.rr, s->tri.grid, s->nrhs, s->sc, s->rho2, st))) return rc;
    } else if (s->mdiag) {
        if ((rc = launch_pcg_axpy2_dot2(s->dtype, true, s->n, s->d, s->x, s->q, s->r, s->mdiag, s->n, nullptr, s->nrhs, s->part_rz,
                                        s->part_rr, s->vgrid, st, m_pitch(s)))) return rc;
        if ((rc = launch_pcg_delta0(s->dtype, s->part_rz, s->part_rr, s->vgrid, s->nrhs, s->sc, s->rho2, st))) return rc;
    } else {
        CG_HIP(hipMemcpyAsync(s->d, s->r, vbytes, hipMemcpyDeviceToDevice, st));
        if ((rc = launch_dot_partials(s->dtype, s->n, s->r, s->r, s->n, s->nrhs, s->part_rr, s->vgrid, st))) return rc;
        if ((rc = launch_cg_delta0(s->dtype, s->part_rr, s->vgrid, s->nrhs, s->sc, st))) return rc;
    }
    if (!on_device) CG_HIP(hipStreamSynchronize(st));
    s->rhs_set = true;
    s->iters = 0;
    return CGAMD_OK;
}
int cgamd_solver_set_rhs(cgamd_solver *s, const void *b, const void *x0, int on_device) {
    if (!s || !b) return fail(CGAMD_ERR_INVALID, "set_rhs: null argument");
    return set_rhs_impl(s, b, x0, on_device, s->n_user);
}

// ... 753 lines not shown
    if (!s->herm) return fail(CGAMD_ERR_STATE, "hermitian_scalars: the handle does not run the conjugated recurrence (use cgamd_solver_step_state)");
    if (int rc = step_not_capturing(s, "hermitian_scalars")) return rc;
    CG_HIP(hipSetDevice(s->ctx->device));
    const size_t bytes = dtype_size(s->dtype) * (size_t)s->nrhs;
    if (alpha_host) CG_HIP(hipMemcpyAsync(alpha_host, s->sc.alpha, bytes, hipMemcpyDeviceToHost, s->ctx->stream));
    if (beta_host) CG_HIP(hipMemcpyAsync(beta_host, s->sc.beta, bytes, hipMemcpyDeviceToHost, s->ctx->stream));
    CG_HIP(hipStreamSynchronize(s->ctx->stream));
    return CGAMD_OK;
}

int cgamd_solver_spmm_rowmajor(cgamd_solver *s, const void *x, void *y, int nRHS) {
    if (!s || !x || !y) return fail(CGAMD_ERR_INVALID, "spmm_rowmajor: null argument");
    if (s->nsys) return fail(CGAMD_ERR_STATE, "spmm_rowmajor: the handle is batched (a matrix of its own per right-hand side)");
    TuneScope ts(&s->tune);
    CG_HIP(hipSetDevice(s->ctx->device));
    return launch_spmm_rm(s->dtype, s->n_user, s->nnz, s->vals, s->ptr, s->cols, x, y, nRHS, nullptr, s->plan.max_quad, s->rm_pace, s->ctx->stream);
}

int cgamd_solver_layout(cgamd_solver *s) { return s ? (s->rm ? 1 : 0) : -CGAMD_ERR_INVALID; }
int cgamd_solver_loop_launches(cgamd_solver *s) {
    if (!s) return -CGAMD_ERR_INVALID;
    TuneScope ts(&s->tune);
    if (s->herm) return 4;
    if (s->mg) return 5 + mg_cost(s->mg).launches;
    if (s->tri_on) return s->tri.longform ? 6 : 4;
    if (s->nsys && s->mdiag) return 4;
    if (s->flags & CGAMD_UNFUSED) return 8;
    if (s->rm) return 5;
    if (s->mdiag) return (s->resw.ok && !s->rm && !(s->flags & (CGAMD_NO_GRAPH | CGAMD_UNFUSED))) ? 1 : 4;
    if (fused2_now(s) && s->res_ok && !(s->flags & CGAMD_NO_GRAPH)) return 0;
    if (s->resw.ok && !(s->flags & CGAMD_NO_GRAPH)) return 1;
    if (fused2_now(s)) return 2;
    return fold_alpha_ok(s->plan.n_partials, s->plan.fold_max) ? 3 : 4;
}

int cgamd_solver_x_lag(cgamd_solver *s) {
    if (!s) return -CGAMD_ERR_INVALID;
    return x_lag_now(s);
}

int cgamd_solver_index_codes(cgamd_solver *s) { return s ? s->n_offsets : -CGAMD_ERR_INVALID; }

static long long value_arrays(const cgamd_solver *s) { return s->nsys ? s->nsys : 1; }
long long cgamd_solver_spmv_bytes(cgamd_solver *s) {
    if (!s) return 0;
    const long long V = (long long)dtype_size(s->dtype);
    return s->nnz * (value_arrays(s) * V + 4) + ((long long)s->n_user + 1) * 4 + 2LL * s->n_user * V * s->nrhs;
}
static long long mg_bytes(const cgamd_solver *s, long long spmv_bytes) {
    const MgCost c = mg_cost(s->mg);
    return 12LL * s->n_user * (long long)dtype_size(s->dtype) * s->nrhs + c.spmv0 * spmv_bytes + c.bytes;
}
static long long tri_passes(const cgamd_solver *s) {
    const long long f = value_arrays(s);
    if (s->tri.stride > 1) return 14LL * s->nrhs + 3 * f;
    return s->tri.longform ? 13LL * s->nrhs + 6 * f : 11LL * s->nrhs + 3 * f;
}
long long cgamd_solver_iter_bytes(cgamd_solver *s, int fused) {
    if (!s) return 0;
    const long long V = (long long)dtype_size(s->dtype);
    if (s->mg) return s->nnz * (V + 4) + ((long long)s->n_user + 1) * 4 + mg_bytes(s, cgamd_solver_spmv_bytes(s));
    if (s->tri_on) return s->nnz * (value_arrays(s) * V + 4) + ((long long)s->n_user + 1) * 4 + tri_passes(s) * s->n_user * V;
    if (s->herm) return s->nnz * (value_arrays(s) * V + 4) + ((long long)s->n_user + 1) * 4 + (s->mdiag ? 14LL : 12LL) * s->n_user * V * s->nrhs;
    if (s->nsys && s->mdiag) return s->nnz * (value_arrays(s) * V + 4) + ((long long)s->n_user + 1) * 4 + 12LL * s->n_user * V * s->nrhs;
    return s->nnz * (value_arrays(s) * V + 4) + ((long long)s->n_user + 1) * 4 + (fused ? 11LL : 14LL) * s->n_user * V * s->nrhs;
}

static long long index_bytes_per_nnz(const cgamd_solver *s) { return s->plan.codes ? (s->plan.codes16 ? 2 : 1) : 4; }
static bool joint_form(const cgamd_solver *s) {
    const int fit = s->plan.max_row <= 0 ? 8 : s->plan.max_row <= 4 ? 4 : s->plan.max_row == 5 ? 5 : s->plan.max_row <= 7 ? 7 : 8;
    return s->plan.jcodes && s->nrhs == 1 && s->plan.max_row > 0 && s->plan.max_row <= fit && dtype_size(s->dtype) <= 8;
}
static bool row_form(const cgamd_solver *s) { return joint_form(s) && s->plan.rcodes && s->plan.rcodes_for == s->ptr && s->tune.dev_row_codes != 0 && s->tune.dev_vc_pipe != 0; }
long long cgamd_solver_spmv_moved_bytes(cgamd_solver *s) {
    if (!s) return 0;
    const long long V = (long long)dtype_size(s->dtype);
    if (row_form(s)) return (long long)s->n_user + 2LL * s->n_user * V;
    const long long value_bytes = joint_form(s) ? 0 : s->plan.vcodes ? 1 : V * value_arrays(s);
    return s->nnz * (value_bytes + index_bytes_per_nnz(s)) + ((long long)s->n_user + 1) * 4 + 2LL * s->n_user * V * s->nrhs;
}
int cgamd_solver_value_codes(cgamd_solver *s) { return s ? s->n_values : -CGAMD_ERR_INVALID; }
int cgamd_solver_joint_codes(cgamd_solver *s) { return s ? (joint_form(s) ? s->n_pairs : 0) : -CGAMD_ERR_INVALID; }
int cgamd_solver_row_codes(cgamd_solver *s) { return s ? (row_form(s) ? s->n_user_patterns : 0) : -CGAMD_ERR_INVALID; }
int cgamd_solver_row_pipe(cgamd_solver *s) { return s ? (row_form(s) ? row_pipe_depth(s->tune.dev_row_pipe, dtype_size(s->dtype)) : 0) : -CGAMD_ERR_INVALID; }
long long cgamd_solver_iter_moved_bytes(cgamd_solver *s) {
    if (!s) return 0;
    const long long V = (long long)dtype_size(s->dtype);
    const long long passes = s->herm ? (s->mdiag ? 14 : 12) : (s->nsys && s->mdiag) ? 12 : (s->flags & CGAMD_UNFUSED) ? 14 : s->mdiag ? 12 : 10;
    const long long lag = x_lag_now(s);
    const long long value_bytes = joint_form(s) ? 0 : s->plan.vcodes ? 1 : V * value_arrays(s);
    const long long matrix = row_form(s) ? (long long)s->n_user : s->nnz * (value_bytes + index_bytes_per_nnz(s)) + ((long long)s->n_user + 1) * 4;
    if (s->mg) return matrix + mg_bytes(s, cgamd_solver_spmv_moved_bytes(s));
    if (s->tri_on) return matrix + tri_passes(s) * s->n_user * V;
    if (lag >= 2) return matrix + (9 * lag + 1) * s->n_user * V * s->nrhs / lag;
    return matrix + passes * s->n_user * V * s->nrhs;
}

}

namespace cgamd {
const void *solver_matrix(cgamd_solver *s, const int **ptr, const int **cols) {
    *ptr = s->ptr; *cols = s->cols;
    return s->vals;
}
int solver_restart(cgamd_solver *s) {
    if (!s->rhs_set) return fail(CGAMD_ERR_STATE, "mixed_solve: the outer handle has no right-hand side");
    return set_rhs_impl(s, nullptr, nullptr, 1, s->n);
}
int solver_set_rhs_ld(cgamd_solver *s, const void *b, long long ldb) { return set_rhs_impl(s, b, nullptr, 1, ldb); }
int solver_replace_residual_ld(cgamd_solver *s, const void *r_new, long long ldr) { return replace_residual_impl(s, r_new, ldr); }
int solver_replace_planned(cgamd_solver *s) {
    TuneScope ts(&s->tune);
    return replace_refuses(s, true);
}
}
```

conjugate-gradient-pyopencl_amd/csrc/spmv.hip:

```cpp
#include "cgamd_internal.h"
#include "device_types.h"
#include "device_mem.h"
#include "spmv_device.h"
#include "reduce_device.h"
#include "launch_util.h"

#include <hip/hip_ext.h>

#include <algorithm>
#include <functional>
#include <mutex>
#include <vector>

namespace cgamd {

template <typename T, int BLOCK, int QPT, bool VEC, bool FUSE_DOT>
__global__ __launch_bounds__(BLOCK) void spmv_stream_kernel(SpmvArgs<T> a) {
    using A = typename VT<T>::acc;
    constexpr int CHUNK = 4 * QPT * BLOCK;
    __shared__ T prod[CHUNK];
    __shared__ A red[BLOCK / kWave];
    extern __shared__ __attribute__((aligned(16))) char dyn_smem[];
    A *wavedot = reinterpret_cast<A *>(dyn_smem);

// ... 483 lines not shown
constexpr int kRowSlots = 7;
template <typename T, int BLOCK, bool NT, bool FUSE_DOT, int DEPTH>
__global__ __launch_bounds__(BLOCK) void spmv_rowcode_kernel(RowcodeArgs<T> a) {
    using A = typename VT<T>::acc;
    extern __shared__ __attribute__((aligned(16))) char dyn_smem[];
    __shared__ A red[kVcBlocks][BLOCK / kWave];
    static_assert(BLOCK == 256, "row blocks of 256 rows");
    static_assert(DEPTH == 1 || DEPTH == 2 || DEPTH == 4, "blocks in flight");
    const int t = threadIdx.x, lane = t & (kWave - 1), wave = t / kWave;
    const int supers = (a.row_blocks + kVcBlocks - 1) / kVcBlocks;
    const int srb = rowblock_of(blockIdx.x, supers, a.cycle);
    if (srb < 0) return;
    const int rb0 = srb * kVcBlocks, nb = min(kVcBlocks, a.row_blocks - rb0);
    const int np = a.n_patterns;
    T *sval = reinterpret_cast<T *>(dyn_smem);
    int *soff = reinterpret_cast<int *>(dyn_smem + (size_t)np * 8 * sizeof(T));
    int *slen = soff + np * 8;
    int code[kVcBlocks];
#pragma unroll
    for (int i = 0; i < kVcBlocks; ++i) {
        const int rc = min((rb0 + min(i, nb - 1)) * BLOCK + t, a.n - 1);
        code[i] = NT ? __builtin_nontemporal_load(a.rcodes + rc) : a.rcodes[rc];
    }
    for (int k = t; k < np * 8; k += BLOCK) { sval[k] = a.rdict_val[k]; soff[k] = a.rdict_off[k]; }
    if (t < np) slen[t] = a.rdict_len[t];
    const __amdgpu_buffer_rsrc_t xrs = __builtin_amdgcn_make_buffer_rsrc(const_cast<T *>(a.x), 0, 0x7ffffffc, 0x00020000);
    [[maybe_unused]] const __amdgpu_buffer_rsrc_t xrs_d = __builtin_amdgcn_make_buffer_rsrc(const_cast<T *>(FUSE_DOT ? a.dvec : a.x), 0, 0x7ffffffc, 0x00020000);
    __builtin_amdgcn_s_waitcnt(0);
    __syncthreads();
    struct Gath { T xv[kRowSlots]; T dv; int len; };
    auto issue = [&](int i) -> Gath {
        Gath g;
        const int row = (rb0 + i) * BLOCK + t;
        const unsigned row8 = (unsigned)min(row, a.n - 1) * (unsigned)sizeof(T);
        const int c = code[i];
        g.len = (row < a.n && i < nb) ? slen[c] : 0;
        const i32x4 o0 = *reinterpret_cast<const i32x4 *>(soff + c * 8), o1 = *reinterpret_cast<const i32x4 *>(soff + c * 8 + 4);
        const int po[8] = {o0.x, o0.y, o0.z, o0.w, o1.x, o1.y, o1.z, o1.w};
        g.dv = vzero<T>();
        if (FUSE_DOT) g.dv = buf_gather<T>(xrs_d, row8);
#pragma unroll
        for (int j = 0; j < kRowSlots; ++j) g.xv[j] = buf_gather<T>(xrs, j < g.len ? row8 + (unsigned)po[j] : row8);
        return g;
    };
    [[maybe_unused]] A dotw[kVcBlocks];
    auto consume = [&](int i, const Gath &g) {
        const int row = (rb0 + i) * BLOCK + t;
        const int c = code[i];
        T pv[8];
        {
            using V = typename Chunk16<T>::V;
            constexpr int EPC = 16 / (int)sizeof(T);
#pragma unroll
            for (int k = 0; k < 8 / EPC; ++k) {
                const V v = *reinterpret_cast<const V *>(sval + c * 8 + k * EPC);
                __builtin_memcpy(&pv[k * EPC], &v, 16);
            }
        }
        T sum = vzero<T>();
#pragma unroll
        for (int j = 0; j < kRowSlots; ++j) {
            const T nxt = vfma(pv[j], g.xv[j], sum);
            sum = vsel(j < g.len, nxt, sum);
        }
        A dot1 = vzero<A>();
        if (row < a.n && i < nb) {
            a.y[row] = sum;
            if (FUSE_DOT) dot1 = to_acc(vmul(g.dv, sum));
        }
        if (FUSE_DOT) dotw[i] = wave_sum(dot1);
    };
    Gath g[DEPTH];
#pragma unroll
    for (int i = 0; i < DEPTH; ++i) g[i] = issue(i);
#pragma unroll
    for (int i = 0; i < kVcBlocks; ++i) {
        consume(i, g[i % DEPTH]);
        if (i + DEPTH < kVcBlocks) g[i % DEPTH] = issue(i + DEPTH);
    }
    if (FUSE_DOT) {
        if (lane == 0) {
#pragma unroll
            for (int i = 0; i < kVcBlocks; ++i) red[i][wave] = dotw[i];
        }
        __syncthreads();
        if (t < nb) {
            A v = red[t][0];
#pragma unroll
            for (int w = 1; w < BLOCK / kWave; ++w) v = vadd(v, red[t][w]);
            a.partials[rb0 + t] = v;
        }
    }
}

template <typename T, int BLOCK, bool NT, bool FUSE_DOT, int LPR, int UNROLL, int CODED = 0>
__global__ __launch_bounds__(BLOCK) void spmv_rowblock_chunked_kernel(SpmvArgs<T> a) {
    using A = typename VT<T>::acc;
    extern __shared__ __attribute__((aligned(16))) char dyn_smem[];
    T *sv = reinterpret_cast<T *>(dyn_smem);
    int *sc = reinterpret_cast<int *>(dyn_smem + (size_t)a.cap * sizeof(T));
    __shared__ A red[BLOCK / kWave];
    __shared__ int sdict[CODED == 1 ? BLOCK : 1];
    constexpr int RC = BLOCK / LPR;
    const int t = threadIdx.x, j = t / LPR, l = t % LPR;
    if constexpr (CODED == 1) sdict[t] = a.dict[t];
    const int rb = rowblock_of(blockIdx.x, a.row_blocks, a.cycle);
    if (rb < 0) return;
    [[maybe_unused]] const int cbase = CODED == 2 ? a.dict[rb] : 0;
    A dot1 = vzero<A>();
    for (int c = 0; c < LPR; ++c) {
        const int c0 = rb * BLOCK + c * RC;
        if (c0 >= a.n) break;
        const int row = c0 + j;
        const int rclamp = min(row, a.n - 1);
        const int s_raw = a.ptr[rclamp], e_raw = a.ptr[rclamp + 1];
        const int p0 = a.ptr[c0], p1 = a.ptr[min(c0 + RC, a.n)];
        const int cfirst = p0 & ~3;
        if (c) __syncthreads();
        stage_slice<T, BLOCK, NT, CODED == 1 ? -3 : CODED == 2 ? -4 : -2>(a.vals, a.cols, a.nnz, cfirst, p1, sv, sc, a.codes);
        const int s = s_raw - cfirst, e = (row < a.n) ? e_raw - cfirst : s_raw - cfirst;
        __syncthreads();
        T sum = vzero<T>();
        for (int k = s + l; k < e; k += UNROLL * LPR) {
            T xv[UNROLL], av[UNROLL];
            int cj[UNROLL];
            const int last = k + ((e - 1 - k) / LPR) * LPR;
#pragma unroll
            for (int u = 0; u < UNROLL; ++u) {
                const int idx = min(k + u * LPR, last);
                if constexpr (CODED == 1) cj[u] = reinterpret_cast<const unsigned char *>(sc)[idx];
                else if constexpr (CODED == 2) cj[u] = cbase + reinterpret_cast<const unsigned short *>(sc)[idx];
                else cj[u] = sc[idx];
                av[u] = sv[idx];
            }
            if constexpr (CODED == 1) {
#pragma unroll
                for (int u = 0; u < UNROLL; ++u) cj[u] = row + sdict[cj[u]];
            }
#pragma unroll
            for (int u = 0; u < UNROLL; ++u) xv[u] = a.x[cj[u]];
#pragma unroll
            for (int u = 0; u < UNROLL; ++u) {
                const T nxt = vfma(av[u], xv[u], sum);
                sum = vsel(k + u * LPR < e, nxt, sum);
            }
        }
#pragma unroll
        for (int off = LPR / 2; off > 0; off >>= 1) {
            if constexpr (VT<T>::cplx) {
                sum.x += __shfl_xor(sum.x, off, kWave);
                sum.y += __shfl_xor(sum.y, off, kWave);
            } else {
                sum += __shfl_xor(sum, off, kWave);
            }
        }
        if (l == 0 && row < a.n) {
            a.y[row] = sum;
            if (FUSE_DOT) dot1 = vadd(dot1, to_acc(vmul(a.dvec[row], sum)));
        }
    }
    if (FUSE_DOT) {
        const A tot = block_sum<BLOCK>(dot1, red);
        if (t == 0) a.partials[rb] = tot;
    }
}

// ... 234 lines not shown
static thread_local int t_form[kSpmvFormFields] = {-1, 0, 0, 0, 0, 0, 0, 0, 0, 0};
static inline void record_form(int family, bool vec, int width, int ienc, int venc, bool nt, bool fused, bool wide, unsigned gx, int parts) {
    t_form[0] = family; t_form[1] = vec; t_form[2] = width; t_form[3] = ienc; t_form[4] = venc;
    t_form[5] = nt; t_form[6] = fused; t_form[7] = wide; t_form[8] = (int)gx; t_form[9] = fused ? parts : 0;
}
void last_spmv_form(int *out, int n_out) {
    for (int i = 0; i < n_out && i < kSpmvFormFields; ++i) out[i] = t_form[i];
}
void record_spmv_form(const int *fields) {
    for (int i = 0; i < kSpmvFormFields; ++i) t_form[i] = fields[i];
}

SpmvPlan make_spmv_plan(int n) {
    SpmvPlan p;
    p.row_blocks = (n + kBlock - 1) / kBlock;
    const int cap = tune().spmv_grid > 0 ? tune().spmv_grid : kMaxGrid;
    int g = p.row_blocks < cap ? p.row_blocks : cap;
    if (g >= 8) g &= ~7;
    if (g < 1) g = 1;
    p.grid = g;
    p.n_partials = g;
    return p;
}

template <typename T>
static int spmv_impl(const SpmvPlan &plan, int n, long long nnz, const void *vals, const int *ptr, const int *cols,
                     const void *x, long long ldx, void *y, long long ldy, int nrhs, const void *dvec, void *partials,
                     const int *rb_list, int rb_count, hipStream_t st) {
    SpmvArgs<T> a;
    a.n = n; a.nrhs = nrhs; a.nnz = nnz;
    a.vals = static_cast<const T *>(vals); a.ptr = ptr; a.cols = cols;
    a.x = static_cast<const T *>(x); a.ldx = ldx;
    a.y = static_cast<T *>(y); a.ldy = ldy;
    a.dvec = static_cast<const T *>(dvec);
    a.partials = static_cast<typename VT<T>::acc *>(partials);
    a.row_blocks = plan.row_blocks;
    a.rb_list = rb_list; a.rb_count = rb_count;
    a.codes = nullptr; a.dict = nullptr; a.vcodes = nullptr; a.vdict = nullptr;
    const bool vec = aligned16(vals) && aligned16(cols);
    const bool fuse = partials != nullptr;
    const size_t dyn = (fuse && nrhs > 1) ? sizeof(typename VT<T>::acc) * nrhs * (kBlock / kWave) : 0;
    dim3 grid(plan.grid), block(kBlock);
    const int variant = (vec && ((nrhs == 1 && plan.kind == 5) || (nrhs > 1 && plan.kind == 6 && plan.wide))) ? 5 : 0;
    if (variant == 5) {
        a.cap = (plan.max_span + 3) & ~3;
        a.cycle = tune().spmv_cycle > 0 ? tune().spmv_cycle : 1;
        dim3 g5(rb_list ? (rb_count > 0 ? rb_count : 1) : rowblock_grid(plan.row_blocks, a.cycle), nrhs);
        if (rb_list && rb_count <= 0) return CGAMD_OK;
        const bool nt = tune().spmv_nt >= 0 ? (tune().spmv_nt != 0) : (plan.nt != 0);
        const bool coded_any = nrhs == 1 && plan.codes && plan.codes_for == cols && tune().index_codes != 0;
        const bool coded = coded_any && !plan.codes16, coded16 = coded_any && plan.codes16;
        const bool vcoded = coded && !rb_list && plan.vcodes && plan.vcodes_for == vals && tune().value_codes != 0 && a.cap <= 8 * kBlock && (unsigned long long)n * sizeof(T) < (1ULL << 30);
        a.codes = coded_any ? plan.codes : nullptr;
        a.dict = coded_any ? plan.dict : nullptr;
        const size_t lds = coded ? (((size_t)a.cap * (sizeof(T) + 1) + 15) & ~(size_t)15)
                                 : coded16 ? (((size_t)a.cap * (sizeof(T) + 2) + 15) & ~(size_t)15) : (size_t)a.cap * (sizeof(T) + 4);
#define CG_RB(NT, UNR)                                                                                                  \
    do {                                                                                                                \
        if (coded16) {                                                                                                  \
            record_form(1, true, UNR, 16, 0, NT, fuse, g5.y > 1, g5.x, plan.row_blocks);                                \
            if (fuse) CG_LAUNCH_EV((spmv_rowblock_kernel<T, kBlock, NT, true, UNR, -4>), g5, block, lds, st, a);        \
            else CG_LAUNCH_EV((spmv_rowblock_kernel<T, kBlock, NT, false, UNR, -4>), g5, block, lds, st, a);            \
        } else if (coded) {                                                                                             \
            record_form(1, true, UNR, 8, 0, NT, fuse, g5.y > 1, g5.x, plan.row_blocks);                                 \
            if (fuse) CG_LAUNCH_EV((spmv_rowblock_kernel<T, kBlock, NT, true, UNR, -3>), g5, block, lds, st, a);        \
            else CG_LAUNCH_EV((spmv_rowblock_kernel<T, kBlock, NT, false, UNR, -3>), g5, block, lds, st, a);            \
        } else {                                                                                                        \
            record_form(1, true, UNR, 0, 0, NT, fuse, g5.y > 1, g5.x, plan.row_blocks);                                 \
            if (fuse) CG_LAUNCH_EV((spmv_rowblock_kernel<T, kBlock, NT, true, UNR, -2>), g5, block, lds, st, a);        \
            else CG_LAUNCH_EV((spmv_rowblock_kernel<T, kBlock, NT, false, UNR, -2>), g5, block, lds, st, a);            \
        }                                                                                                               \
    } while (0)
        const int fit = plan.max_row <= 0 ? 8 : plan.max_row <= 4 ? 4 : plan.max_row == 5 ? 5 : plan.max_row <= 7 ? 7 : 8;
        const int unroll = tune().spmv_unroll ? tune().spmv_unroll : (sizeof(T) > 8 ? 4 : fit);
        if constexpr (sizeof(T) <= 8) {
            if (vcoded) {
                a.vcodes = plan.vcodes; a.vdict = static_cast<const T *>(plan.vdict);
                const size_t lds2 = (((size_t)a.cap * 4 * kVcRows + 15) & ~(size_t)15) + 16;
                const int supers = (plan.row_blocks + kVcBlocks - 1) / kVcBlocks, cyc = std::max(1, a.cycle / kVcBlocks);
                a.cycle = cyc;
                const dim3 gvc(rowblock_grid(supers, cyc));
                const bool pipe = plan.max_row > 0 && plan.max_row <= unroll && tune().dev_vc_pipe != 0;
                const bool joint = pipe && plan.jcodes && tune().dev_joint_codes != 0;
                if (joint && plan.rcodes && plan.rcodes_for == ptr && tune().dev_row_codes != 0) {
                    RowcodeArgs<T> ra;
                    ra.n = n; ra.row_blocks = plan.row_blocks; ra.cycle = cyc; ra.n_patterns = plan.n_patterns;
                    ra.x = a.x; ra.y = a.y; ra.dvec = a.dvec; ra.partials = a.partials;
                    ra.rcodes = plan.rcodes; ra.rdict_len = plan.rdict_len; ra.rdict_off = plan.rdict_off;
                    ra.rdict_val = static_cast<const T *>(plan.rdict_val);
                    const size_t ldsr = (size_t)plan.n_patterns * (8 * sizeof(T) + 8 * sizeof(int) + sizeof(int));
                    record_form(7, true, unroll, 8, 3, nt, fuse, false, gvc.x, plan.row_blocks);
#define CG_RC(DEPTH)                                                                                                    \
    do {                                                                                                                \
        if (nt) {                                                                                                       \
            if (fuse) CG_LAUNCH_EV((spmv_rowcode_kernel<T, kBlock, true, true, DEPTH>), gvc, block, ldsr, st, ra);      \
            else CG_LAUNCH_EV((spmv_rowcode_kernel<T, kBlock, true, false, DEPTH>), gvc, block, ldsr, st, ra);          \
        } else {                                                                                                        \
            if (fuse) CG_LAUNCH_EV((spmv_rowcode_kernel<T, kBlock, false, true, DEPTH>), gvc, block, ldsr, st, ra);     \
            else CG_LAUNCH_EV((spmv_rowcode_kernel<T, kBlock, false, false, DEPTH>), gvc, block, ldsr, st, ra);         \
        }                                                                                                               \
    } while (0)
                    const int depth = row_pipe_depth(tune().dev_row_pipe, sizeof(T));
                    if (depth == 1) CG_RC(1);
                    else if (depth == 2) CG_RC(2);
                    else CG_RC(4);
#undef CG_RC
                    return check_launch("spmv_rowcode");
                }
                if (joint) { a.codes = plan.jcodes; a.dict = plan.jdict_off; a.vdict = static_cast<const T *>(plan.jdict_val); a.vcodes = nullptr; }
#define CG_VC(NT, UNR)                                                                                                  \
    do {                                                                                                                \
        if (joint) {                                                                                                    \
            record_form(3, true, UNR, 8, 2, NT, fuse, false, gvc.x, plan.row_blocks);                                   \
            if (fuse) CG_LAUNCH_EV((spmv_rowblock_vcp_kernel<T, kBlock, NT, true, UNR, true>), gvc, block, lds2, st, a); \
            else CG_LAUNCH_EV((spmv_rowblock_vcp_kernel<T, kBlock, NT, false, UNR, true>), gvc, block, lds2, st, a);     \
        } else if (pipe) {                                                                                              \
            record_form(3, true, UNR, 8, 1, NT, fuse, false, gvc.x, plan.row_blocks);                                   \
            if (fuse) CG_LAUNCH_EV((spmv_rowblock_vcp_kernel<T, kBlock, NT, true, UNR, false>), gvc, block, lds2, st, a); \
            else CG_LAUNCH_EV((spmv_rowblock_vcp_kernel<T, kBlock, NT, false, UNR, false>), gvc, block, lds2, st, a);    \
        } else {                                                                                                        \
            record_form(2, true, UNR, 8, 1, NT, fuse, false, gvc.x, plan.row_blocks);                                   \
            if (fuse) CG_LAUNCH_EV((spmv_rowblock_vc_kernel<T, kBlock, NT, true, UNR>), gvc, block, lds2, st, a);       \
            else CG_LAUNCH_EV((spmv_rowblock_vc_kernel<T, kBlock, NT, false, UNR>), gvc, block, lds2, st, a);           \
        }                                                                                                               \
    } while (0)
                if (unroll == 4) { if (nt) CG_VC(true, 4); else CG_VC(false, 4); }
                else if (unroll == 5) { if (nt) CG_VC(true, 5); else CG_VC(false, 5); }
                else if (unroll == 7) { if (nt) CG_VC(true, 7); else CG_VC(false, 7); }
                else { if (nt) CG_VC(true, 8); else CG_VC(false, 8); }
#undef CG_VC
                return check_launch("spmv_rowblock_vc");
            }
        }
        if (unroll == 4) { if (nt) CG_RB(true, 4); else CG_RB(false, 4); }
        else if (unroll == 5) { if (nt) CG_RB(true, 5); else CG_RB(false, 5); }
        else if (unroll == 7) { if (nt) CG_RB(true, 7); else CG_RB(false, 7); }
        else { if (nt) CG_RB(true, 8); else CG_RB(false, 8); }
#undef CG_RB
        return check_launch("spmv_rowblock");
    }
    if (vec && nrhs == 1 && plan.kind == 7 && !rb_list) {
        const int span = plan.chunk_span[plan.lpr == 2 ? 0 : plan.lpr == 4 ? 1 : plan.lpr == 8 ? 2 : plan.lpr == 16 ? 3 : 4];
        a.cap = (span + 3) & ~3;
        a.cycle = tune().spmv_cycle > 0 ? tune().spmv_cycle : 1;
        const bool coded_any = plan.codes && plan.codes_for == cols && tune().index_codes != 0;
        const bool coded = coded_any && !plan.codes16, coded16 = coded_any && plan.codes16;
        a.codes = coded_any ? plan.codes : nullptr;
        a.dict = coded_any ? plan.dict : nullptr;
        const size_t lds = coded ? (((size_t)a.cap * (sizeof(T) + 1) + 15) & ~(size_t)15)
                                 : coded16 ? (((size_t)a.cap * (sizeof(T) + 2) + 15) & ~(size_t)15) : (size_t)a.cap * (sizeof(T) + 4);
        const dim3 g7(rowblock_grid(plan.row_blocks, a.cycle));
        const bool nt = tune().spmv_nt >= 0 ? (tune().spmv_nt != 0) : (plan.nt != 0);
        constexpr int U = sizeof(T) > 8 ? 4 : 8;
#define CG_CH(NT, L)                                                                                                     \
    do {                                                                                                                  \
        if (coded16) {                                                                                                    \
            record_form(4, true, L, 16, 0, NT, fuse, false, g7.x, plan.row_blocks);                                       \
            if (fuse) hipLaunchKernelGGL((spmv_rowblock_chunked_kernel<T, kBlock, NT, true, L, U, 2>), g7, block, lds, st, a);      \
            else hipLaunchKernelGGL((spmv_rowblock_chunked_kernel<T, kBlock, NT, false, L, U, 2>), g7, block, lds, st, a);          \
        } else if (coded) {                                                                                               \
            record_form(4, true, L, 8, 0, NT, fuse, false, g7.x, plan.row_blocks);                                        \
            if (fuse) hipLaunchKernelGGL((spmv_rowblock_chunked_kernel<T, kBlock, NT, true, L, U, 1>), g7, block, lds, st, a);      \
            else hipLaunchKernelGGL((spmv_rowblock_chunked_kernel<T, kBlock, NT, false, L, U, 1>), g7, block, lds, st, a);          \
        } else {                                                                                                          \
            record_form(4, true, L, 0, 0, NT, fuse, false, g7.x, plan.row_blocks);                                        \
            if (fuse) hipLaunchKernelGGL((spmv_rowblock_chunked_kernel<T, kBlock, NT, true, L, U>), g7, block, lds, st, a); \
            else hipLaunchKernelGGL((spmv_rowblock_chunked_kernel<T, kBlock, NT, false, L, U>), g7, block, lds, st, a);   \
// ... 211 lines not shown
```

include/cgamd.h:

```cpp
#ifndef CGAMD_H
#define CGAMD_H
#include <stddef.h>

#ifdef __cplusplus
extern "C" {
#endif

typedef enum { CGAMD_F32 = 0, CGAMD_F64 = 1, CGAMD_C64 = 2, CGAMD_C128 = 3 } cgamd_dtype;

typedef enum {
    CGAMD_OK = 0,
    CGAMD_ERR_INVALID = 1,
    CGAMD_ERR_NO_DEVICE = 2,
    CGAMD_ERR_HIP = 3,
    CGAMD_ERR_ALLOC = 4,
    CGAMD_ERR_IO = 5,
    CGAMD_ERR_COMM = 6,
    CGAMD_ERR_STATE = 7
} cgamd_status;

typedef struct cgamd_ctx cgamd_ctx;
typedef struct cgamd_solver cgamd_solver;

const char *cgamd_last_error(void);
// ... 13 lines not shown

int cgamd_malloc(cgamd_ctx *ctx, size_t bytes, void **dptr);
int cgamd_free(cgamd_ctx *ctx, void *dptr);
int cgamd_memcpy_h2d(cgamd_ctx *ctx, void *dst, const void *src, size_t bytes);
int cgamd_memcpy_d2h(cgamd_ctx *ctx, void *dst, const void *src, size_t bytes);
int cgamd_memcpy_d2d(cgamd_ctx *ctx, void *dst, const void *src, size_t bytes);
int cgamd_memset(cgamd_ctx *ctx, void *dst, int value, size_t bytes);

int cgamd_spmv(cgamd_ctx *ctx, int dtype, int size, long long nnz, const void *aValues,
               const int *aPointers, const int *aCols, const void *x, void *y, int nRHS);
int cgamd_vdot(cgamd_ctx *ctx, int dtype, int size, const void *a, const void *b, void *result, int nRHS);
int cgamd_axpy(cgamd_ctx *ctx, int dtype, int size, const void *x, void *y, const void *a, int aSign, int nRHS);
int cgamd_aypx(cgamd_ctx *ctx, int dtype, int size, const void *x, void *y, const void *a, int nRHS);
int cgamd_sub(cgamd_ctx *ctx, int dtype, int size, const void *a, const void *b, void *result, int nRHS);

#define CGAMD_MATRIX_ON_DEVICE 1
#define CGAMD_NO_GRAPH 2
#define CGAMD_UNFUSED 4
#define CGAMD_HERMITIAN 16
#define CGAMD_DIST_NO_OVERLAP 32
#define CGAMD_DIST_P2P 64
#define CGAMD_DIST_GRAPH 8
#define CGAMD_DIST_P2P_STAGED 128

#define CGAMD_DIST_SINGLE_REDUCTION 256

#define CGAMD_DIST_RESIDENT 512

int cgamd_solver_create(cgamd_ctx *ctx, int dtype, int size, long long nnz, const void *aValues,
                        const int *aPointers, const int *aCols, int nRHS, int flags, cgamd_solver **out);
int cgamd_solver_create_batched(cgamd_ctx *ctx, int dtype, int size, long long nnz, const void *aValues,
                                const int *aPointers, const int *aCols, int nSystems, int flags, cgamd_solver **out);
int cgamd_solver_systems(cgamd_solver *s);
int cgamd_solver_hermitian(cgamd_solver *s);
int cgamd_solver_hermitian_scalars(cgamd_solver *s, void *alpha_host, void *beta_host);
int cgamd_solver_destroy(cgamd_solver *s);
int cgamd_solver_reload_matrix(cgamd_solver *s, const void *aValues, const int *aPointers, const int *aCols);
int cgamd_solver_refresh_values(cgamd_solver *s, const void *aValues, int on_device);
int cgamd_solver_last_refresh(cgamd_solver *s);
int cgamd_solver_graph_captures(cgamd_solver *s);
int cgamd_solver_set_rhs(cgamd_solver *s, const void *b, const void *x0, int on_device);
int cgamd_solver_iterate(cgamd_solver *s, int nIterations);
int cgamd_solver_iterate_tol(cgamd_solver *s, int maxIterations, double tol, int *iterations_run);
int cgamd_solver_iterate_until(cgamd_solver *s, int maxIterations, const double *tol, int nTol, int checkEvery, int *iterations_run);
int cgamd_solver_replace_residual(cgamd_solver *s, const void *r_new);
int cgamd_solver_iterate_timed(cgamd_solver *s, int nIterations, float *spmv_ms_avg, float *iter_ms_avg);
int cgamd_solver_get_x(cgamd_solver *s, void *x, int on_device);
int cgamd_solver_history(cgamd_solver *s, void *history, int max_entries);
int cgamd_solver_iterations_done(cgamd_solver *s);
void *cgamd_solver_vector(cgamd_solver *s, int which);
int cgamd_solver_ld(cgamd_solver *s);
int cgamd_solver_set_preconditioner(cgamd_solver *s, const void *m, int on_device);
int cgamd_solver_set_preconditioner_tridiag(cgamd_solver *s, const void *lower, const void *diag, const void *upper, int on_device);
int cgamd_solver_set_preconditioner_tridiag_strided(cgamd_solver *s, int stride, const void *lower, const void *diag,
                                                    const void *upper, int on_device);
int cgamd_solver_set_preconditioner_line(cgamd_solver *s, int stride);
int cgamd_solver_set_preconditioner_jacobi(cgamd_solver *s);
int cgamd_solver_set_preconditioner_batched(cgamd_solver *s, const void *m, int on_device);
int cgamd_solver_set_preconditioner_batched_jacobi(cgamd_solver *s);
int cgamd_solver_set_preconditioner_batched_line(cgamd_solver *s, int stride);
int cgamd_solver_set_preconditioner_multigrid(cgamd_solver *s, int nx, int ny, int nz, int smooth_steps, double over_correction, int min_rows);
int cgamd_solver_mg_levels(cgamd_solver *s);
int cgamd_solver_mg_level(cgamd_solver *s, int level, long long info[6]);
int cgamd_solver_mg_level_matrix(cgamd_solver *s, int level, int *ptr, int *cols, void *vals);
int cgamd_solver_mg_apply(cgamd_solver *s, const void *r_dev, void *z_dev);
int cgamd_solver_set_preconditioner_amg(cgamd_solver *s, int passes, double strength, int smooth_steps, double over_correction, int min_rows);
int cgamd_solver_mg_aggregates(cgamd_solver *s, int level, int *agg_host, int *n_coarse);
int cgamd_solver_preconditioner_source(cgamd_solver *s);
int cgamd_solver_solve(cgamd_solver *s, const void *b, void *x, int nIterations, void *history);
int cgamd_solver_spmv(cgamd_solver *s, const void *x, void *y, int fused_dot);
int cgamd_last_spmv_form(int *out, int n_out);
int cgamd_solver_dot_partials(cgamd_solver *s, void *out_host, long long cap_values, int *per_rhs);
int cgamd_solver_step_plan(cgamd_solver *s, int *out, int n_out);
int cgamd_solver_step_state(cgamd_solver *s, int which, void *out_host, long long cap_values, long long *count);
int cgamd_solver_spmm_rowmajor(cgamd_solver *s, const void *x, void *y, int nRHS);
int cgamd_solver_layout(cgamd_solver *s);
int cgamd_solver_loop_launches(cgamd_solver *s);
int cgamd_solver_x_lag(cgamd_solver *s);
int cgamd_solver_index_codes(cgamd_solver *s);
int cgamd_solver_value_codes(cgamd_solver *s);
int cgamd_solver_joint_codes(cgamd_solver *s);
int cgamd_solver_row_codes(cgamd_solver *s);
int cgamd_solver_row_pipe(cgamd_solver *s);
int cgamd_transpose(cgamd_ctx *ctx, int dtype, int rows, int cols, const void *in, void *out);
long long cgamd_solver_spmv_bytes(cgamd_solver *s);
long long cgamd_solver_iter_bytes(cgamd_solver *s, int fused);
long long cgamd_solver_spmv_moved_bytes(cgamd_solver *s);
long long cgamd_solver_iter_moved_bytes(cgamd_solver *s);

typedef struct cgamd_mixed cgamd_mixed;
int cgamd_mixed_create(cgamd_ctx *ctx, int dtype_hi, int size, long long nnz, const void *aValues_hi, const int *aPointers,
                       const int *aCols, int nRHS, int flags, cgamd_mixed **out);
int cgamd_mixed_destroy(cgamd_mixed *m);
cgamd_solver *cgamd_mixed_outer(cgamd_mixed *m);
cgamd_solver *cgamd_mixed_inner(cgamd_mixed *m);
int cgamd_mixed_solve(cgamd_mixed *m, const void *b, void *x, int on_device, const double *tol, int nTol, int maxIterations, double delta,
                      int maxSegment, int checkEvery, int *iterations, double *resnorm, int *status, int *replacements);
int cgamd_mixed_scales(cgamd_mixed *m, double *scales);

int cgamd_cg(int dtype, int size, long long nnz, const void *aValues, const void *b, const int *aPointers,
             const int *aCols, void *x, int nRHS, int nIterations, void *history, int device);
int cgamd_cg_last_timing(double *ms6);
int cgamd_cg_release_cache(void);

int cgamd_gen_laplace3d(cgamd_ctx *ctx, int dtype, int nx, int ny, int nz, long long row_begin,
                        long long row_end, void *aValues, int *aPointers, int *aCols, long long *nnz_out);
int cgamd_gen_poisson2d(cgamd_ctx *ctx, int dtype, int N, void *aValues, int *aPointers, int *aCols,
                        long long *nnz_out);

int cgamd_gen_helm_fe_var(cgamd_ctx *ctx, int dtype, int N, double omega, const double *C, double rho, int Nhoriz, int Nvert,
                          void *aValues, int *aPointers, int *aCols, long long *nnz_out);
int cgamd_gen_local_rect(cgamd_ctx *ctx, int dtype, int N, double k, double eps, double eta, double L, int Nhoriz, int Nvert,
                         void *aValues, int *aPointers, int *aCols, long long *nnz_out);

int cgamd_gen_rhs(cgamd_ctx *ctx, int dtype, int kind, int N, double k, void *b);

int cgamd_mm_read(const char *path, int *size, long long *nnz, int *is_complex, double **values,
                  int **pointers, int **cols);
void cgamd_mm_free(void *p);

typedef struct cgamd_dist cgamd_dist;
int cgamd_comm_unique_id(void *id128);
int cgamd_dist_create(cgamd_ctx *ctx, const void *id128, int rank, int nranks, int dtype,
                      int n_local, int n_halo, long long nnz_local, const void *aValues,
                      const int *aPointers, const int *aCols,
                      int n_peers, const int *peer_rank, const int *send_count, const int *recv_count,
                      const int *send_index ,
                      int flags, cgamd_dist **out);
int cgamd_dist_destroy(cgamd_dist *d);
int cgamd_dist_set_rhs(cgamd_dist *d, const void *b_local, const void *x0_local);
int cgamd_dist_iterate(cgamd_dist *d, int nIterations);
int cgamd_dist_iterate_until(cgamd_dist *d, int maxIterations, double tol, int checkEvery, int *iterations_run);
int cgamd_dist_iterations_done(cgamd_dist *d);
int cgamd_dist_get_x(cgamd_dist *d, void *x_local);
int cgamd_dist_history(cgamd_dist *d, void *history, int max_entries);
int cgamd_dist_synchronize(cgamd_dist *d);
int cgamd_dist_set_preconditioner(cgamd_dist *d, const void *m_local);
int cgamd_dist_set_preconditioner_jacobi(cgamd_dist *d);
int cgamd_dist_set_preconditioner_line(cgamd_dist *d, int stride);
int cgamd_dist_refresh_values(cgamd_dist *d);
int cgamd_dist_last_refresh(cgamd_dist *d);
int cgamd_p2p_mailbox_alloc(cgamd_ctx *ctx, long long halo_values, int dtype, void **mailbox, void *handle64);
int cgamd_p2p_mailbox_free(cgamd_ctx *ctx, void *mailbox);
int cgamd_dist_attach_p2p(cgamd_dist *d, void *my_mailbox, const void *handles, const int *dst_offset);
int cgamd_dist_p2p_error(cgamd_dist *d);
int cgamd_dist_enable_resident(cgamd_dist *d, long long mailbox_values, const int *rank_n_local, const int *rank_n_halo);
int cgamd_dist_index_codes(cgamd_dist *d);
int cgamd_dist_loop_launches(cgamd_dist *d);
int cgamd_dist_comm_ranks(cgamd_dist *d);

#ifdef __cplusplus
}
#endif
#endif
```

Measured before the change: 6877 CG iterations/s.

## Add row-pair pattern codes SpMV kernel merging adjacent rows' stencil slots

Builds a second-level dictionary that encodes each pair of adjacent rows by a one-byte code mapping to a merged union of column offsets (LCS-merged, up to 8 slots), with per-row value tables. A new SpMV kernel has each thread process two rows and gather both x values for each union slot with a single 2-wide buffer load. It also writes y as a 16-byte pair. This halves the code-stream bytes per row and the gather instruction count. In exchange it adds a setup pass, an LDS-staged dictionary and extra select/masked FMA work. It is enabled by default for f64 when the row-code form is active.

```diff
diff --git a/conjugate-gradient-pyopencl_amd/_lib.py b/conjugate-gradient-pyopencl_amd/_lib.py
--- a/conjugate-gradient-pyopencl_amd/_lib.py
+++ b/conjugate-gradient-pyopencl_amd/_lib.py
@@ -111,6 +111,7 @@
         "cgamd_solver_joint_codes": (ci, [vp]),
         "cgamd_solver_row_codes": (ci, [vp]),
         "cgamd_solver_row_pipe": (ci, [vp]),
+        "cgamd_solver_row_pairs": (ci, [vp]),
         "cgamd_solver_iterate_tol": (ci, [vp, ci, ctypes.c_double, ctypes.POINTER(ci)]),
         "cgamd_solver_iterate_until": (ci, [vp, ci, ctypes.POINTER(ctypes.c_double), ci, ci, ctypes.POINTER(ci)]),
         "cgamd_solver_replace_residual": (ci, [vp, vp]),
diff --git a/conjugate-gradient-pyopencl_amd/cl.py b/conjugate-gradient-pyopencl_amd/cl.py
--- a/conjugate-gradient-pyopencl_amd/cl.py
+++ b/conjugate-gradient-pyopencl_amd/cl.py
@@ -453,7 +453,7 @@
         check(self._lib.cgamd_solver_spmv(self.handle, ptr(x), ptr(y), int(fused_dot)))
 
     SPMV_FAMILIES = ("stream", "rowblock", "vc", "vcp", "chunked", "spmm", "batched")
-    SPMV_FAMILIES_EXTRA = ("rowcode",)
+    SPMV_FAMILIES_EXTRA = ("rowcode", "rowpair")
     SPMV_FORM_FIELDS = ("family", "vec", "width", "index_bits", "value_codes", "nt", "fused", "wide", "grid", "partials")
 
     def last_spmv_form(self):
@@ -535,6 +535,10 @@
     @property
     def row_pipe(self):
         return self._lib.cgamd_solver_row_pipe(self.handle)
+
+    @property
+    def row_pairs(self):
+        return self._lib.cgamd_solver_row_pairs(self.handle)
 
     def iter_bytes(self, fused=False):
         return self._lib.cgamd_solver_iter_bytes(self.handle, int(fused))
diff --git a/conjugate-gradient-pyopencl_amd/csrc/api.cpp b/conjugate-gradient-pyopencl_amd/csrc/api.cpp
--- a/conjugate-gradient-pyopencl_amd/csrc/api.cpp
+++ b/conjugate-gradient-pyopencl_amd/csrc/api.cpp
@@ -38,6 +38,8 @@
         return fail(CGAMD_ERR_INVALID, "tune: dev.x_lag takes -1 (default rule), 0 or 1 (off), 2, 4 or 8");
     if (k == "dev.row_pipe" && value != 0 && value != 1 && value != 2 && value != 4)
         return fail(CGAMD_ERR_INVALID, "tune: dev.row_pipe takes 0 (default rule), 1, 2 or 4");
+    if (k == "dev.row_pairs" && value != -1 && value != 0 && value != 1)
+        return fail(CGAMD_ERR_INVALID, "tune: dev.row_pairs takes -1 (default rule), 0 or 1");
     g_tune_generation.fetch_add(1, std::memory_order_relaxed);
     tune_set([&](Tuning &g_tune) {
     if (k == "index_codes") g_tune.index_codes = value;
@@ -65,6 +67,8 @@
     else if (k == "dev.row_codes") g_tune.dev_row_codes = value;
     else if (k == "dev.row_codes_min_mb") g_tune.dev_row_codes_min_mb = value;
     else if (k == "dev.row_pipe") g_tune.dev_row_pipe = value;
+    else if (k == "dev.row_pairs") g_tune.dev_row_pairs = value;
+    else if (k == "dev.row_pairs_min_mb") g_tune.dev_row_pairs_min_mb = value;
     else if (k == "dev.resident_lock") g_tune.resident_lock = value;
     else if (k == "dev.slab_cus") g_tune.slab_cus = value;
     else if (k == "dev.slab_trim") g_tune.slab_trim = value;
diff --git a/conjugate-gradient-pyopencl_amd/csrc/cgamd_internal.h b/conjugate-gradient-pyopencl_amd/csrc/cgamd_internal.h
--- a/conjugate-gradient-pyopencl_amd/csrc/cgamd_internal.h
+++ b/conjugate-gradient-pyopencl_amd/csrc/cgamd_internal.h
@@ -58,6 +58,10 @@
     const void *rdict_val = nullptr;
     int n_patterns = 0;
     const int *rcodes_for = nullptr;
+    const unsigned char *pcodes = nullptr;
+    const void *pdict = nullptr;
+    int n_pair_patterns = 0;
+    int pair_slots = 0;
 };
 SpmvPlan make_spmv_plan(int n);
 int compute_spmv_plan(const int *ptr_dev, const int *cols_dev, int n, int *scratch_dev, hipStream_t st, SpmvPlan *plan);
@@ -74,6 +78,16 @@
 constexpr size_t row_dict_alloc_bytes(size_t value_size) { return row_dict_jmap_at(value_size) + 256 * 8; }
 int build_row_codes(int dtype, int n, int n_user, const int *ptr_dev, const unsigned char *jcodes, const int *joff, const void *jval, hipStream_t st,
                     unsigned char **rcodes_out, void **rdict_out, int *n_patterns, int *n_user_patterns);
+constexpr size_t pair_dict_val1_at(int np, size_t value_size) { return (size_t)np * 8 * value_size; }
+constexpr size_t pair_dict_off_at(int np, size_t value_size) { return 2 * (size_t)np * 8 * value_size; }
+constexpr size_t pair_dict_mask_at(int np, size_t value_size) { return pair_dict_off_at(np, value_size) + (size_t)np * 8 * sizeof(int); }
+constexpr size_t pair_dict_stage_bytes(int np, size_t value_size) { return pair_dict_mask_at(np, value_size) + (size_t)np * sizeof(int); }
+constexpr size_t pair_dict_src_at(int np, size_t value_size) { return pair_dict_stage_bytes(np, value_size); }
+constexpr size_t pair_dict_alloc_bytes(int np, size_t value_size) { return pair_dict_src_at(np, value_size) + (size_t)np * 16 * sizeof(unsigned short); }
+constexpr size_t kPairDictLdsCap = 16 * 1024;
+int build_row_pairs(int dtype, int n, const unsigned char *rcodes, const void *rdict, int n_patterns, hipStream_t st,
+                    unsigned char **pcodes_out, void **pdict_out, int *n_pair_patterns, int *max_slots);
+int refresh_pair_dict(int dtype, int n_pair_patterns, const void *rdict, void *pdict, hipStream_t st);
 int build_value_codes(int dtype, long long nnz, const void *vals_dev, hipStream_t st, unsigned char **vcodes_out, void **vdict_out, int *n_values);
 int refresh_value_dicts(int dtype, long long nnz, const void *vals_dev, const unsigned char *vcodes, void *vdict, int n_pairs, const int *joff,
                         void *jval, int n_patterns, void *rdict, hipStream_t st, bool *kept);
@@ -108,6 +122,8 @@
     int dev_row_codes = 1;
     int dev_row_codes_min_mb = 32;
     int dev_row_pipe = 0;
+    int dev_row_pairs = -1;
+    int dev_row_pairs_min_mb = 256;
     int dev_vc_pipe = 1;
     int dev_generic_spmv = 0;
     int resident_lock = 1;
@@ -131,6 +147,7 @@
     int dev_line_host_route = 0;
 };
 inline int row_pipe_depth(int knob, size_t value_bytes) { return knob == 1 || knob == 2 || knob == 4 ? knob : value_bytes <= 4 ? 4 : 1; }
+inline bool row_pairs_wanted(int knob, size_t value_bytes) { return knob == 1 ? true : knob == 0 ? false : value_bytes >= 8; }
 extern Tuning g_tune;
 Tuning tune_snapshot();
 const Tuning &tune();
diff --git a/conjugate-gradient-pyopencl_amd/csrc/index_codes.hip b/conjugate-gradient-pyopencl_amd/csrc/index_codes.hip
--- a/conjugate-gradient-pyopencl_amd/csrc/index_codes.hip
+++ b/conjugate-gradient-pyopencl_amd/csrc/index_codes.hip
@@ -4,6 +4,7 @@
 #include "spmv_device.h"
 #include "reduce_device.h"
 #include "launch_util.h"
+#include "row_pairs.h"
 
 #include <hip/hip_ext.h>
 
@@ -613,4 +614,127 @@
     return refresh_value_dicts_impl<float2>(nnz, vals_dev, vcodes, vdict, n_pairs, joff, jval, n_patterns, rdict, st, kept);
 }
 
-}
+constexpr int kPairEmpty = 256;
+constexpr int kPairCombos = 256 * 257;
+__global__ __launch_bounds__(256) void rowpair_mark_kernel(int n, const unsigned char *__restrict__ rcodes, unsigned char *present) {
+    const long long npairs = ((long long)n + 1) / 2, stride = (long long)gridDim.x * 256;
+    for (long long p = (long long)blockIdx.x * 256 + threadIdx.x; p < npairs; p += stride) {
+        const int c0 = rcodes[2 * p], c1 = 2 * p + 1 < n ? (int)rcodes[2 * p + 1] : kPairEmpty;
+        if (!present[c0 * 257 + c1]) present[c0 * 257 + c1] = 1;
+    }
+}
+__global__ __launch_bounds__(256) void rowpair_encode_kernel(int n, const unsigned char *__restrict__ rcodes, const unsigned char *__restrict__ combo_code,
+                                                             unsigned char *__restrict__ pcodes) {
+    const long long npairs = ((long long)n + 1) / 2, stride = (long long)gridDim.x * 256;
+    for (long long p = (long long)blockIdx.x * 256 + threadIdx.x; p < npairs; p += stride) {
+        const int c0 = rcodes[2 * p], c1 = 2 * p + 1 < n ? (int)rcodes[2 * p + 1] : kPairEmpty;
+        pcodes[p] = combo_code[c0 * 257 + c1];
+    }
+}
+template <typename W>
+__global__ __launch_bounds__(256) void rowpair_values_kernel(int np, const W *__restrict__ rval, const unsigned short *__restrict__ src, W *val0, W *val1) {
+    for (int k = threadIdx.x; k < np * 16; k += 256) {
+        const int p = k >> 4, u = k & 7;
+        const unsigned s = src[k];
+        const W v = s == 0xffffu ? (W)0 : rval[s];
+        ((k & 8) ? val1 : val0)[p * 8 + u] = v;
+    }
+}
+static void launch_rowpair_values(size_t vs, int np, const void *rdict, char *pdict, hipStream_t st) {
+    const auto *src = reinterpret_cast<const unsigned short *>(pdict + pair_dict_src_at(np, vs));
+    if (vs == 4)
+        hipLaunchKernelGGL((rowpair_values_kernel<unsigned>), dim3(1), dim3(256), 0, st, np, static_cast<const unsigned *>(rdict), src,
+                           reinterpret_cast<unsigned *>(pdict), reinterpret_cast<unsigned *>(pdict + pair_dict_val1_at(np, vs)));
+    else
+        hipLaunchKernelGGL((rowpair_values_kernel<unsigned long long>), dim3(1), dim3(256), 0, st, np, static_cast<const unsigned long long *>(rdict), src,
+                           reinterpret_cast<unsigned long long *>(pdict), reinterpret_cast<unsigned long long *>(pdict + pair_dict_val1_at(np, vs)));
+}
+int build_row_pairs(int dtype, int n, const unsigned char *rcodes, const void *rdict, int n_patterns, hipStream_t st,
+                    unsigned char **pcodes_out, void **pdict_out, int *n_pair_patterns, int *max_slots) {
+    *pcodes_out = nullptr; *pdict_out = nullptr; *n_pair_patterns = 0; *max_slots = 0;
+    if (n < 2 || !rcodes || !rdict || n_patterns < 1 || dtype == CGAMD_C128) return CGAMD_OK;
+    const size_t vs = dtype_size(dtype);
+    unsigned char *marks = nullptr;
+    CG_HIP(hipMalloc((void **)&marks, 2 * (size_t)kPairCombos));
+    std::vector<unsigned char> present(kPairCombos), combo_code(kPairCombos, 0);
+    std::vector<int> roff(256 * 8), rlen(256);
+    const int grid = (int)std::min<long long>((((long long)n + 1) / 2 + 255) / 256, 4096);
+    hipError_t e = hipMemsetAsync(marks, 0, kPairCombos, st);
+    if (e == hipSuccess) {
+        hipLaunchKernelGGL(rowpair_mark_kernel, dim3(grid), dim3(256), 0, st, n, rcodes, marks);
+        e = hipMemcpyAsync(present.data(), marks, kPairCombos, hipMemcpyDeviceToHost, st);
+    }
+    const char *rd = static_cast<const char *>(rdict);
+    if (e == hipSuccess) e = hipMemcpyAsync(roff.data(), rd + row_dict_off_at(vs), 256 * 8 * sizeof(int), hipMemcpyDeviceToHost, st);
+    if (e == hipSuccess) e = hipMemcpyAsync(rlen.data(), rd + row_dict_len_at(vs), 256 * sizeof(int), hipMemcpyDeviceToHost, st);
+    if (e == hipSuccess) e = hipStreamSynchronize(st);
+    std::vector<PairPattern> pats;
+    std::vector<int> combos;
+    bool fits = e == hipSuccess;
+    for (int c = 0; fits && c < kPairCombos; ++c) {
+        if (!present[c]) continue;
+        const int c0 = c / 257, c1 = c % 257;
+        if (pats.size() == 256 || c0 >= n_patterns || (c1 != kPairEmpty && c1 >= n_patterns)) { fits = false; break; }
+        const int len0 = rlen[c0], len1 = c1 == kPairEmpty ? 0 : rlen[c1];
+        PairPattern pp;
+        if (!merge_pair_slots(len0, &roff[c0 * 8], len1, c1 == kPairEmpty ? nullptr : &roff[c1 * 8], &pp)) { fits = false; break; }
+        combo_code[c] = (unsigned char)pats.size();
+        pats.push_back(pp);
+        combos.push_back(c);
+    }
+    const int np = (int)pats.size();
+    if (fits && (np < 1 || pair_dict_stage_bytes(np, vs) > kPairDictLdsCap)) fits = false;
+    unsigned char *pcodes = nullptr;
+    char *pdict = nullptr;
+    int slots = 0;
+    for (const PairPattern &pp : pats) slots = std::max(slots, pp.n);
+    if (fits) {
+        std::vector<char> img(pair_dict_alloc_bytes(np, vs), 0);
+        int *off = reinterpret_cast<int *>(img.data() + pair_dict_off_at(np, vs));
+        int *mask = reinterpret_cast<int *>(img.data() + pair_dict_mask_at(np, vs));
+        auto *src = reinterpret_cast<unsigned short *>(img.data() + pair_dict_src_at(np, vs));
+        for (int p = 0; p < np; ++p) {
+            const int c0 = combos[p] / 257, c1 = combos[p] % 257;
+            int m = 0;
+            for (int u = 0; u < kPairSlots; ++u) {
+                const PairPattern &pp = pats[p];
+                off[p * 8 + u] = u < pp.n ? pp.off[u] : 0;
+                const bool use0 = u < pp.n && pp.src0[u] >= 0, use1 = u < pp.n && pp.src1[u] >= 0;
+                src[p * 16 + u] = use0 ? (unsigned short)(c0 * 8 + pp.src0[u]) : (unsigned short)0xffffu;
+                src[p * 16 + 8 + u] = use1 ? (unsigned short)(c1 * 8 + pp.src1[u]) : (unsigned short)0xffffu;
+                m |= (use0 ? 1 << u : 0) | (use1 ? 256 << u : 0);
+            }
+            mask[p] = m;
+        }
+        e = hipMalloc((void **)&pcodes, ((size_t)n + 1) / 2 + 64);
+        if (e == hipSuccess) e = hipMalloc((void **)&pdict, img.size());
+        if (e == hipSuccess) e = hipMemsetAsync(pcodes + ((size_t)n + 1) / 2, 0, 64, st);
+        if (e == hipSuccess) e = hipMemcpyAsync(pdict, img.data(), img.size(), hipMemcpyHostToDevice, st);
+        if (e == hipSuccess) e = hipMemcpyAsync(marks + kPairCombos, combo_code.data(), kPairCombos, hipMemcpyHostToDevice, st);
+        if (e == hipSuccess) {
+            launch_rowpair_values(vs, np, rdict, pdict, st);
+            hipLaunchKernelGGL(rowpair_encode_kernel, dim3(grid), dim3(256), 0, st, n, rcodes, marks + kPairCombos, pcodes);
+            e = hipGetLastError();
+        }
+        if (e == hipSuccess) e = hipStreamSynchronize(st);
+    }
+    (void)hipFree(marks);
+    if (e != hipSuccess) {
+        if (pcodes) (void)hipFree(pcodes);
+        if (pdict) (void)hipFree(pdict);
+        return fail(CGAMD_ERR_HIP, std::string("build_row_pairs: ") + hipGetErrorString(e));
+    }
+    *pcodes_out = pcodes; *pdict_out = pdict; *n_pair_patterns = fits ? np : 0;
+    if (fits) *max_slots = slots;
+    return CGAMD_OK;
+}
+int refresh_pair_dict(int dtype, int n_pair_patterns, const void *rdict, void *pdict, hipStream_t st) {
+    if (!rdict || !pdict || n_pair_patterns < 1 || dtype == CGAMD_C128) return CGAMD_OK;
+    launch_rowpair_values(dtype_size(dtype), n_pair_patterns, rdict, static_cast<char *>(pdict), st);
+    hipError_t e = hipGetLastError();
+    if (e == hipSuccess) e = hipStreamSynchronize(st);
+    if (e != hipSuccess) return fail(CGAMD_ERR_HIP, std::string("refresh_pair_dict: ") + hipGetErrorString(e));
+    return CGAMD_OK;
+}
+
+}
diff --git a/conjugate-gradient-pyopencl_amd/csrc/row_pairs.cpp b/conjugate-gradient-pyopencl_amd/csrc/row_pairs.cpp
--- /dev/null
+++ b/conjugate-gradient-pyopencl_amd/csrc/row_pairs.cpp
@@ -0,0 +1,30 @@
+#include "row_pairs.h"
+
+namespace cgamd {
+
+bool merge_pair_slots(int len0, const int *off0, int len1, const int *off1, PairPattern *out) {
+    constexpr int M = 8;
+    out->n = 0;
+    for (int u = 0; u < kPairSlots; ++u) { out->off[u] = 0; out->src0[u] = -1; out->src1[u] = -1; }
+    if (len0 < 0 || len1 < 0 || len0 > M || len1 > M) { out->n = kPairSlots + 1; return false; }
+    int lcs[M + 1][M + 1];
+    for (int i = len0; i >= 0; --i)
+        for (int j = len1; j >= 0; --j) {
+            if (i == len0 || j == len1) lcs[i][j] = 0;
+            else if (off0[i] == off1[j]) lcs[i][j] = lcs[i + 1][j + 1] + 1;
+            else lcs[i][j] = lcs[i + 1][j] >= lcs[i][j + 1] ? lcs[i + 1][j] : lcs[i][j + 1];
+        }
+    const int total = len0 + len1 - lcs[0][0];
+    if (total > kPairSlots) { out->n = total; return false; }
+    int i = 0, j = 0, u = 0;
+    while (i < len0 || j < len1) {
+        if (i < len0 && j < len1 && off0[i] == off1[j]) { out->off[u] = off0[i]; out->src0[u] = i++; out->src1[u] = j++; }
+        else if (j == len1 || (i < len0 && lcs[i + 1][j] >= lcs[i][j + 1])) { out->off[u] = off0[i]; out->src0[u] = i++; }
+        else { out->off[u] = off1[j]; out->src1[u] = j++; }
+        ++u;
+    }
+    out->n = u;
+    return true;
+}
+
+}
diff --git a/conjugate-gradient-pyopencl_amd/csrc/row_pairs.h b/conjugate-gradient-pyopencl_amd/csrc/row_pairs.h
--- /dev/null
+++ b/conjugate-gradient-pyopencl_amd/csrc/row_pairs.h
@@ -0,0 +1,13 @@
+#pragma once
+
+namespace cgamd {
+
+constexpr int kPairSlots = 8;
+
+struct PairPattern {
+    int n;
+    int off[kPairSlots], src0[kPairSlots], src1[kPairSlots];
+};
+bool merge_pair_slots(int len0, const int *off0, int len1, const int *off1, PairPattern *out);
+
+}
diff --git a/conjugate-gradient-pyopencl_amd/csrc/solver.cpp b/conjugate-gradient-pyopencl_amd/csrc/solver.cpp
--- a/conjugate-gradient-pyopencl_amd/csrc/solver.cpp
+++ b/conjugate-gradient-pyopencl_amd/csrc/solver.cpp
@@ -72,6 +72,9 @@
     int n_pairs = 0;
     unsigned char *rcodes = nullptr;
     void *rdict = nullptr;
+    unsigned char *pcodes = nullptr;
+    void *pdict = nullptr;
+    int n_pair_patterns = 0;
     int n_patterns = 0, n_user_patterns = 0;
     double tol_req = 0.;
     bool tol_served = false, tol_stopped = false;
@@ -302,6 +305,10 @@
     s->plan.rcodes = nullptr; s->plan.rdict_len = nullptr; s->plan.rdict_off = nullptr; s->plan.rdict_val = nullptr; s->plan.n_patterns = 0;
     s->plan.rcodes_for = nullptr;
     s->n_patterns = 0; s->n_user_patterns = 0;
+    if (s->pcodes) { (void)hipFree(s->pcodes); s->pcodes = nullptr; }
+    if (s->pdict) { (void)hipFree(s->pdict); s->pdict = nullptr; }
+    s->plan.pcodes = nullptr; s->plan.pdict = nullptr; s->plan.n_pair_patterns = 0; s->plan.pair_slots = 0;
+    s->n_pair_patterns = 0;
 }
 static bool value_codes_apply(const cgamd_solver *s) {
     return s->codes && !s->plan.codes16 && !s->nsys && s->tune.value_codes && s->plan.kind == 5 && s->dtype != CGAMD_C128;
@@ -327,6 +334,12 @@
             s->plan.rdict_off = reinterpret_cast<const int *>(rd + row_dict_off_at(vsz));
             s->plan.rdict_len = reinterpret_cast<const int *>(rd + row_dict_len_at(vsz));
             s->plan.rcodes_for = s->ptr;
+            if (row_pairs_wanted(s->tune.dev_row_pairs, vsz) && s->tune.dev_row_pairs_min_mb >= 0 &&
+                matrix_bytes > ((size_t)s->tune.dev_row_pairs_min_mb << 20)) {
+                if (int rc = build_row_pairs(s->dtype, s->n, s->rcodes, s->rdict, s->n_patterns, s->ctx->stream, &s->pcodes, &s->pdict,
+                                             &s->n_pair_patterns, &s->plan.pair_slots)) return rc;
+                if (s->pcodes) { s->plan.pcodes = s->pcodes; s->plan.pdict = s->pdict; s->plan.n_pair_patterns = s->n_pair_patterns; }
+            }
         }
     }
     return CGAMD_OK;
@@ -682,6 +695,13 @@
             drop_value_codes(s);
             return rc;
         }
+        if (kept && s->pdict) {
+            if (int rc = refresh_pair_dict(s->dtype, s->n_pair_patterns, s->rdict, s->pdict, s->ctx->stream)) {
+                destroy_graphs(s);
+                drop_value_codes(s);
+                return rc;
+            }
+        }
         if (kept) { s->last_refresh = 1; return CGAMD_OK; }
     }
     const bool had = s->vcodes != nullptr;
@@ -754,7 +774,7 @@
         if (s->cols) (void)hipFree(s->cols);
     }
     void *bufs[] = {s->slab, s->part_dq, s->part_rr, s->sc.alpha, s->sc.beta, s->sc.delta,
-                    s->sc.history, s->sc.iter, s->mdiag, s->part_rz, s->rho2, s->tri_coef, s->tri_part, s->tri_cstart, s->tri.maps, s->sc.stage, s->sc.ticket, s->res_sync, s->resw_sync, s->dlag, s->codes, s->dict, s->rm_pace, s->vcodes, s->vdict, s->jcodes, s->jdict_off, s->jdict_val, s->rcodes, s->rdict};
+                    s->sc.history, s->sc.iter, s->mdiag, s->part_rz, s->rho2, s->tri_coef, s->tri_part, s->tri_cstart, s->tri.maps, s->sc.stage, s->sc.ticket, s->res_sync, s->resw_sync, s->dlag, s->codes, s->dict, s->rm_pace, s->vcodes, s->vdict, s->jcodes, s->jdict_off, s->jdict_val, s->rcodes, s->rdict, s->pcodes, s->pdict};
     for (void *p : bufs)
         if (p) (void)hipFree(p);
     stop_run_free(s->stop);
@@ -1674,6 +1694,10 @@
 int cgamd_solver_value_codes(cgamd_solver *s) { return s ? s->n_values : -CGAMD_ERR_INVALID; }
 int cgamd_solver_joint_codes(cgamd_solver *s) { return s ? (joint_form(s) ? s->n_pairs : 0) : -CGAMD_ERR_INVALID; }
 int cgamd_solver_row_codes(cgamd_solver *s) { return s ? (row_form(s) ? s->n_user_patterns : 0) : -CGAMD_ERR_INVALID; }
+int cgamd_solver_row_pairs(cgamd_solver *s) {
+    if (!s) return -CGAMD_ERR_INVALID;
+    return row_form(s) && s->plan.pcodes && row_pairs_wanted(s->tune.dev_row_pairs, dtype_size(s->dtype)) ? s->n_pair_patterns : 0;
+}
 int cgamd_solver_row_pipe(cgamd_solver *s) { return s ? (row_form(s) ? row_pipe_depth(s->tune.dev_row_pipe, dtype_size(s->dtype)) : 0) : -CGAMD_ERR_INVALID; }
 long long cgamd_solver_iter_moved_bytes(cgamd_solver *s) {
     if (!s) return 0;
diff --git a/conjugate-gradient-pyopencl_amd/csrc/spmv.hip b/conjugate-gradient-pyopencl_amd/csrc/spmv.hip
--- a/conjugate-gradient-pyopencl_amd/csrc/spmv.hip
+++ b/conjugate-gradient-pyopencl_amd/csrc/spmv.hip
@@ -589,6 +589,151 @@
         if (lane == 0) {
 #pragma unroll
             for (int i = 0; i < kVcBlocks; ++i) red[i][wave] = dotw[i];
+        }
+        __syncthreads();
+        if (t < nb) {
+            A v = red[t][0];
+#pragma unroll
+            for (int w = 1; w < BLOCK / kWave; ++w) v = vadd(v, red[t][w]);
+            a.partials[rb0 + t] = v;
+        }
+    }
+}
+
+template <typename T> struct RowpairArgs {
+    int n, row_blocks, cycle, n_pair_patterns;
+    const T *x;
+    T *y;
+    const T *dvec;
+    typename VT<T>::acc *partials;
+    const unsigned char *pcodes;
+    const void *pdict;
+};
+template <typename T> struct Two { T a, b; };
+template <typename T> CG_DEV Two<T> buf_gather2(__amdgpu_buffer_rsrc_t rs, unsigned byte_off) {
+    Two<T> r;
+    if constexpr (sizeof(T) == 4) {
+        const u32x2 w = __builtin_amdgcn_raw_buffer_load_b64(rs, byte_off, 0, 0);
+        __builtin_memcpy(&r, &w, 8);
+    } else {
+        const u32x4 w = __builtin_amdgcn_raw_buffer_load_b128(rs, byte_off, 0, 0);
+        __builtin_memcpy(&r, &w, 16);
+    }
+    return r;
+}
+CG_DEV double half_wave_sum(double v) {
+    const unsigned long long b0 = (unsigned long long)__double_as_longlong(v);
+    v = __longlong_as_double((long long)(((b0 >> 32) << 32) | exec_settle((unsigned)b0)));
+    v += lanes_plus16(v);
+    v += dpp_row_shl<8>(v);
+    v += dpp_row_shl<4>(v);
+    v += dpp_row_shl<2>(v);
+    v += dpp_row_shl<1>(v);
+    return v;
+}
+CG_DEV double2 half_wave_sum(double2 v) { return make_double2(half_wave_sum(v.x), half_wave_sum(v.y)); }
+constexpr int kPairPasses = kVcBlocks / 2;
+template <typename T, int BLOCK, bool NT, bool FUSE_DOT, int DEPTH, int SLOTS>
+__global__ __launch_bounds__(BLOCK) void spmv_rowpair_kernel(RowpairArgs<T> a) {
+    using A = typename VT<T>::acc;
+    extern __shared__ __attribute__((aligned(16))) char dyn_smem[];
+    __shared__ A red[kVcBlocks][BLOCK / kWave];
+    static_assert(BLOCK == 256 && kVcBlocks == 4, "two passes of 512 rows");
+    static_assert(DEPTH == 1 || DEPTH == 2, "passes in flight");
+    static_assert(SLOTS == 7 || SLOTS == 8, "union slots");
+    const int t = threadIdx.x, lane = t & (kWave - 1), wave = t / kWave;
+    const int supers = (a.row_blocks + kVcBlocks - 1) / kVcBlocks;
+    const int srb = rowblock_of(blockIdx.x, supers, a.cycle);
+    if (srb < 0) return;
+    const int rb0 = srb * kVcBlocks, nb = min(kVcBlocks, a.row_blocks - rb0);
+    const int np = a.n_pair_patterns;
+    const T *sval0 = reinterpret_cast<const T *>(dyn_smem), *sval1 = sval0 + np * 8;
+    const int *soff = reinterpret_cast<const int *>(sval1 + np * 8), *smask = soff + np * 8;
+    const int npairs = (a.n + 1) / 2;
+    int code[kPairPasses];
+#pragma unroll
+    for (int p = 0; p < kPairPasses; ++p) {
+        const int q = min(rb0 * (BLOCK / 2) + p * BLOCK + t, npairs - 1);
+        code[p] = NT ? __builtin_nontemporal_load(a.pcodes + q) : a.pcodes[q];
+    }
+    {
+        const int words = np * (16 * (int)sizeof(T) + 8 * (int)sizeof(int) + (int)sizeof(int)) / 4;
+        const int *src = static_cast<const int *>(a.pdict);
+        int *dst = reinterpret_cast<int *>(dyn_smem);
+        for (int k = t; k < words; k += BLOCK) dst[k] = src[k];
+    }
+    const __amdgpu_buffer_rsrc_t xrs = __builtin_amdgcn_make_buffer_rsrc(const_cast<T *>(a.x), 0, 0x7ffffffc, 0x00020000);
+    [[maybe_unused]] const __amdgpu_buffer_rsrc_t xrs_d = __builtin_amdgcn_make_buffer_rsrc(const_cast<T *>(FUSE_DOT ? a.dvec : a.x), 0, 0x7ffffffc, 0x00020000);
+    __builtin_amdgcn_s_waitcnt(0);
+    __syncthreads();
+    const int top = (a.n - 2) * (int)sizeof(T);
+    struct Gath { Two<T> xv[SLOTS]; Two<T> dv; unsigned lo, hi; };
+    auto issue = [&](int p) -> Gath {
+        Gath g;
+        const int base = ((rb0 + 2 * p) * BLOCK + 2 * t) * (int)sizeof(T);
+        const int c = code[p];
+        const i32x4 o0 = *reinterpret_cast<const i32x4 *>(soff + c * 8), o1 = *reinterpret_cast<const i32x4 *>(soff + c * 8 + 4);
+        const int po[8] = {o0.x, o0.y, o0.z, o0.w, o1.x, o1.y, o1.z, o1.w};
+        g.lo = 0; g.hi = base > top ? 1u << 8 : 0u;
+        g.dv.a = vzero<T>(); g.dv.b = vzero<T>();
+        if (FUSE_DOT) g.dv = buf_gather2<T>(xrs_d, (unsigned)min(base, top));
+#pragma unroll
+        for (int u = 0; u < SLOTS; ++u) {
+            const int sb = base + po[u];
+            g.lo |= sb < 0 ? 1u << u : 0u;
+            g.hi |= sb > top ? 1u << u : 0u;
+            g.xv[u] = buf_gather2<T>(xrs, (unsigned)min(max(sb, 0), top));
+        }
+        return g;
+    };
+    [[maybe_unused]] A dotw[kPairPasses];
+    auto consume = [&](int p, const Gath &g) {
+        const int row0 = (rb0 + 2 * p) * BLOCK + 2 * t;
+        const int c = code[p];
+        const int mask = smask[c];
+        T v0[8], v1[8];
+        {
+            using V = typename Chunk16<T>::V;
+            constexpr int EPC = 16 / (int)sizeof(T);
+#pragma unroll
+            for (int k = 0; k < 8 / EPC; ++k) {
+                const V w0 = *reinterpret_cast<const V *>(sval0 + c * 8 + k * EPC), w1 = *reinterpret_cast<const V *>(sval1 + c * 8 + k * EPC);
+                __builtin_memcpy(&v0[k * EPC], &w0, 16);
+                __builtin_memcpy(&v1[k * EPC], &w1, 16);
+            }
+        }
+        T sum0 = vzero<T>(), sum1 = vzero<T>();
+#pragma unroll
+        for (int u = 0; u < SLOTS; ++u) {
+            const T x0 = vsel((g.hi >> u) & 1u, g.xv[u].b, g.xv[u].a);
+            const T x1 = vsel((g.lo >> u) & 1u, g.xv[u].a, g.xv[u].b);
+            const T n0 = vfma(v0[u], x0, sum0), n1 = vfma(v1[u], x1, sum1);
+            sum0 = vsel((mask >> u) & 1, n0, sum0);
+            sum1 = vsel((mask >> (8 + u)) & 1, n1, sum1);
+        }
+        A dot0 = vzero<A>(), dot1 = vzero<A>();
+        if (row0 + 1 < a.n) {
+            if constexpr (sizeof(T) == 4) { u32x2 w; __builtin_memcpy(&w, &sum0, 4); __builtin_memcpy(reinterpret_cast<char *>(&w) + 4, &sum1, 4); *reinterpret_cast<u32x2 *>(a.y + row0) = w; }
+            else { u32x4 w; __builtin_memcpy(&w, &sum0, 8); __builtin_memcpy(reinterpret_cast<char *>(&w) + 8, &sum1, 8); *reinterpret_cast<u32x4 *>(a.y + row0) = w; }
+            if (FUSE_DOT) { dot0 = to_acc(vmul(g.dv.a, sum0)); dot1 = to_acc(vmul(g.dv.b, sum1)); }
+        } else if (row0 < a.n) {
+            a.y[row0] = sum0;
+            if (FUSE_DOT) dot0 = to_acc(vmul(vsel((g.hi >> 8) & 1u, g.dv.b, g.dv.a), sum0));
+        }
+        if (FUSE_DOT) dotw[p] = vadd(half_wave_sum(dot0), half_wave_sum(dot1));
+    };
+    Gath g[DEPTH];
+#pragma unroll
+    for (int p = 0; p < DEPTH; ++p) g[p] = issue(p);
+#pragma unroll
+    for (int p = 0; p < kPairPasses; ++p) {
+        consume(p, g[p % DEPTH]);
+        if (p + DEPTH < kPairPasses) g[p % DEPTH] = issue(p + DEPTH);
+    }
+    if (FUSE_DOT) {
+        if ((lane & 31) == 0) {
+#pragma unroll
+            for (int p = 0; p < kPairPasses; ++p) red[2 * p + (wave >> 1)][2 * (wave & 1) + (lane >> 5)] = dotw[p];
         }
         __syncthreads();
         if (t < nb) {
@@ -989,7 +1134,32 @@
                 const dim3 gvc(rowblock_grid(supers, cyc));
                 const bool pipe = plan.max_row > 0 && plan.max_row <= unroll && tune().dev_vc_pipe != 0;
                 const bool joint = pipe && plan.jcodes && tune().dev_joint_codes != 0;
-                if (joint && plan.rcodes && plan.rcodes_for == ptr && tune().dev_row_codes != 0) {
+                const bool rowform = joint && plan.rcodes && plan.rcodes_for == ptr && tune().dev_row_codes != 0;
+                if (rowform && plan.pcodes && plan.pdict && plan.n_pair_patterns > 0 && row_pairs_wanted(tune().dev_row_pairs, sizeof(T)) && n >= 2 &&
+                    aligned16(a.x) && aligned16(a.y) && (!fuse || aligned16(a.dvec))) {
+                    RowpairArgs<T> pa;
+                    pa.n = n; pa.row_blocks = plan.row_blocks; pa.cycle = cyc; pa.n_pair_patterns = plan.n_pair_patterns;
+                    pa.x = a.x; pa.y = a.y; pa.dvec = a.dvec; pa.partials = a.partials;
+                    pa.pcodes = plan.pcodes; pa.pdict = plan.pdict;
+                    const size_t ldsp = pair_dict_stage_bytes(plan.n_pair_patterns, sizeof(T));
+                    record_form(8, true, unroll, 8, 3, nt, fuse, false, gvc.x, plan.row_blocks);
+#define CG_RP(DEPTH, SLOTS)                                                                                             \
+    do {                                                                                                                \
+        if (nt) {                                                                                                \
+            if (fuse) CG_LAUNCH_EV((spmv_rowpair_kernel<T, kBlock, true, true, DEPTH, SLOTS>), gvc, block, ldsp, st, pa);   \
+            else CG_LAUNCH_EV((spmv_rowpair_kernel<T, kBlock, true, false, DEPTH, SLOTS>), gvc, block, ldsp, st, pa);       \
+        } else {                                                                                                        \
+            if (fuse) CG_LAUNCH_EV((spmv_rowpair_kernel<T, kBlock, false, true, DEPTH, SLOTS>), gvc, block, ldsp, st, pa);  \
+            else CG_LAUNCH_EV((spmv_rowpair_kernel<T, kBlock, false, false, DEPTH, SLOTS>), gvc, block, ldsp, st, pa);      \
+        }                                                                                                               \
+    } while (0)
+                    const int depth = std::min(2, row_pipe_depth(tune().dev_row_pipe, sizeof(T)));
+                    if (plan.pair_slots <= 7) { if (depth == 1) CG_RP(1, 7); else CG_RP(2, 7); }
+                    else { if (depth == 1) CG_RP(1, 8); else CG_RP(2, 8); }
+#undef CG_RP
+                    return check_launch("spmv_rowpair");
+                }
+                if (rowform) {
                     RowcodeArgs<T> ra;
                     ra.n = n; ra.row_blocks = plan.row_blocks; ra.cycle = cyc; ra.n_patterns = plan.n_patterns;
                     ra.x = a.x; ra.y = a.y; ra.dvec = a.dvec; ra.partials = a.partials;
diff --git a/include/cgamd.h b/include/cgamd.h
--- a/include/cgamd.h
+++ b/include/cgamd.h
@@ -119,6 +119,7 @@
 int cgamd_solver_joint_codes(cgamd_solver *s);
 int cgamd_solver_row_codes(cgamd_solver *s);
 int cgamd_solver_row_pipe(cgamd_solver *s);
+int cgamd_solver_row_pairs(cgamd_solver *s);
 int cgamd_transpose(cgamd_ctx *ctx, int dtype, int rows, int cols, const void *in, void *out);
 long long cgamd_solver_spmv_bytes(cgamd_solver *s);
 long long cgamd_solver_iter_bytes(cgamd_solver *s, int fused);
```

Measured after the change: 7560 CG iterations/s, median of 6. 9.9% higher.
